# sshaoshuai/PointRCNN

Measured on AMD Instinct MI355X. Metric: KITTI frames/sec, RPN inference end-to-end (16384 pts/frame, bs32 per GPU), higher is better.
Workload: dtype f32 via split-bf16x6 MFMA (every fp32 operand cut exactly into 3 bf16 pieces, 6 bf16 MFMA products per fp32 product, fp32 accumulate: fp32-grade, measured error 2.9e-7 of sum|x||w| vs 3.0e-7 for the fp32-MFMA kernel; hoisted grouped layers on the split kernel too, unhoisted grouped first layers (xyz; 1 GPU; Full RPN PointNet++ backbone (4 SA-MSG + 4 FP) + cls/reg heads, tools/cfgs/default.yaml, 16384 pts/frame, batch 32 per GPU, random-init weights, eval-mode BN; frames_per_gpu=32, npoints=16384, parallelism=frames sharded, dp1, launch=hipGraph replay, streams=20, hw_queues=4, proposal_layer=normal, clouds=uniform, group_dedup=True, roi_dedup=True

## Files before the change

pointrcnn_amd/csrc/grid.hip:

```cpp
#include "grid_layout.h"

#define GRID_BUILD_THREADS 1024

__device__ __forceinline__ const int32_t* grid_cells(const void* g, size_t fb, int b) { return (const int32_t*)((const char*)g + fb * b + sizeof(GridHeader)); }
__device__ __forceinline__ const float4* grid_points(const void* g, size_t fb, int b) {
    size_t off = (sizeof(GridHeader) + (size_t)(GRID_CELLS_MAX + 1) * 4 + 15) & ~(size_t)15;
    return (const float4*)((const char*)g + fb * b + off);
}

__device__ __forceinline__ int cell_coord(float v, float o, float inv, int dim) {
    float t = (v - o) * inv;
    t = fminf(fmaxf(t, 0.0f), (float)(dim - 1));
    return (int)t;
}

__device__ __forceinline__ float block_reduce(float v, bool is_min, float* scratch) {
    const int lane = threadIdx.x & 63, wave = threadIdx.x >> 6, nw = blockDim.x >> 6;
#pragma unroll
    for (int d = 32; d >= 1; d >>= 1) {
        float o = __shfl_xor(v, d, 64);
        v = is_min ? fminf(v, o) : fmaxf(v, o);
    }
    __syncthreads();
    if (lane == 0) scratch[wave] = v;
    __syncthreads();
    float r = scratch[0];
    for (int w = 1; w < nw; w++) r = is_min ? fminf(r, scratch[w]) : fmaxf(r, scratch[w]);
    return r;
}

__device__ __forceinline__ float block_reduce_sum(float v, float* scratch) {
    const int lane = threadIdx.x & 63, wave = threadIdx.x >> 6, nw = blockDim.x >> 6;
#pragma unroll
    for (int d = 32; d >= 1; d >>= 1) v += __shfl_xor(v, d, 64);
    __syncthreads();
    if (lane == 0) scratch[wave] = v;
    __syncthreads();
    float r = 0.f;
    for (int w = 0; w < nw; w++) r += scratch[w];
    __syncthreads();
    return r;
}

__global__ __launch_bounds__(GRID_BUILD_THREADS) void grid_build_kernel(const float* __restrict__ xyz, int N, float min_cell, int dim,
                                                                        void* grid, size_t fb) {
    extern __shared__ int cnt[];
    const int ncell = dim * dim, per_thread = ncell / GRID_BUILD_THREADS;
    __shared__ float red[16];
    __shared__ int wsum[16];
    const int b = blockIdx.x, tid = threadIdx.x;
    const float* __restrict__ p = xyz + (size_t)b * N * 3;
    GridHeader* H = (GridHeader*)grid_header(grid, fb, b);
    int32_t* cstart = (int32_t*)grid_cells(grid, fb, b);
    float4* sorted = (float4*)grid_points(grid, fb, b);
    float mnx = INFINITY, mxx = -INFINITY, mnz = INFINITY, mxz = -INFINITY;
    for (int i = tid; i < N; i += GRID_BUILD_THREADS) {
        float x = p[i * 3], z = p[i * 3 + 2];
        if (fabsf(x) < INFINITY && fabsf(z) < INFINITY) {
            mnx = fminf(mnx, x); mxx = fmaxf(mxx, x); mnz = fminf(mnz, z); mxz = fmaxf(mxz, z);
        }
    }
    mnx = block_reduce(mnx, true, red); mxx = block_reduce(mxx, false, red);
    mnz = block_reduce(mnz, true, red); mxz = block_reduce(mxz, false, red);
    if (!(mnx <= mxx)) { mnx = mxx = 0.f; mnz = mxz = 0.f; }
    float cs = fmaxf(fmaxf(mxx - mnx, mxz - mnz) / (float)dim * 1.0001f, fmaxf(min_cell, 1e-3f));
    const float inv = 1.0f / cs;
    for (int c = tid; c < ncell; c += GRID_BUILD_THREADS) cnt[c] = 0;
    __syncthreads();
    for (int i = tid; i < N; i += GRID_BUILD_THREADS) {
        int c = cell_coord(p[i * 3 + 2], mnz, inv, dim) * dim + cell_coord(p[i * 3], mnx, inv, dim);
        atomicAdd(&cnt[c], 1);
    }
    __syncthreads();
    int ssum = 0, occ = 0;
    for (int u = 0; u < per_thread; u++) {
        const int c = cnt[tid * per_thread + u];
        ssum += c;
        occ += c > 0;
    }
    const float occupied = block_reduce_sum((float)occ, red);
    int inc = ssum;
    const int lane = tid & 63, wave = tid >> 6;
#pragma unroll
    for (int d = 1; d < 64; d <<= 1) {
        int o = __shfl_up(inc, d, 64);
        if (lane >= d) inc += o;
    }
    if (lane == 63) wsum[wave] = inc;
    __syncthreads();
    int woff = 0;
    for (int w = 0; w < wave; w++) woff += wsum[w];
    int run = woff + inc - ssum;
    for (int u = 0; u < per_thread; u++) {
        const int c = cnt[tid * per_thread + u];
        cstart[tid * per_thread + u] = run;
        cnt[tid * per_thread + u] = run;
        run += c;
    }
    if (tid == GRID_BUILD_THREADS - 1) cstart[ncell] = run;
    if (tid == 0) {
        H->x0 = mnx; H->z0 = mnz; H->inv_cs = inv; H->cs = cs; H->dim = dim;
        const float side = 2.0f * min_cell * inv + 1.0f;
        H->cand = (float)N / fmaxf(occupied, 1.0f) * side * side;
        H->pad1 = H->pad2 = 0;
    }
    __syncthreads();
    for (int i = tid; i < N; i += GRID_BUILD_THREADS) {
        float x = p[i * 3], y = p[i * 3 + 1], z = p[i * 3 + 2];
        int c = cell_coord(z, mnz, inv, dim) * dim + cell_coord(x, mnx, inv, dim);
        int pos = atomicAdd(&cnt[c], 1);
        sorted[pos] = make_float4(x, y, z, __int_as_float(i));
    }
}

#define GBQ_THREADS 64

__device__ __forceinline__ int insert_sorted(int* list, int stride, int cnt, int cap, int k) {
    if (cnt == cap) {
        if (k >= list[(cap - 1) * stride]) return cnt;
        cnt = cap - 1;
    }
    int pos = cnt;
    while (pos > 0 && list[(pos - 1) * stride] > k) { list[pos * stride] = list[(pos - 1) * stride]; pos--; }
    list[pos * stride] = k;
    return cnt + 1;
}

template <bool DUAL>
__global__ __launch_bounds__(GBQ_THREADS) void grid_ball_query_kernel(const void* __restrict__ grid, size_t fb,
                                                                     const float* __restrict__ new_xyz, int M, float ra,
                                                                     float r2a, int nsa, int32_t* __restrict__ idxa, float rb,
                                                                     float r2b, int nsb, int32_t* __restrict__ idxb, int N,
                                                                     int skip_dense) {
    extern __shared__ int lists[];
    const int b = blockIdx.y, tid = threadIdx.x;
    const int m = blockIdx.x * GBQ_THREADS + tid;
    if (m >= M) return;
    const GridHeader H = *grid_header(grid, fb, b);
    if (skip_dense && grid_frame_dense(H, N)) return;
    const int32_t* __restrict__ cstart = grid_cells(grid, fb, b);
    const float4* __restrict__ pts = grid_points(grid, fb, b);
    const float* q = new_xyz + ((size_t)b * M + m) * 3;
    const float qx = q[0], qy = q[1], qz = q[2];
    int* la = lists + tid;
    int* lb = lists + nsa * GBQ_THREADS + tid;
    int cnta = 0, cntb = 0;
    const float rmax = DUAL ? fmaxf(ra, rb) : ra;
    const float r2max = DUAL ? fmaxf(r2a, r2b) : r2a;
    const float rs = rmax * 1.001f + 1e-6f;
    if (qx == qx && qz == qz && r2max > 0.0f) {
        const int dim = H.dim;
        const int cx0 = cell_coord(qx - rs, H.x0, H.inv_cs, dim), cx1 = cell_coord(qx + rs, H.x0, H.inv_cs, dim);
        const int cz0 = cell_coord(qz - rs, H.z0, H.inv_cs, dim), cz1 = cell_coord(qz + rs, H.z0, H.inv_cs, dim);
        for (int cz = cz0; cz <= cz1; cz++) {
            const int beg = cstart[cz * dim + cx0], end = cstart[cz * dim + cx1 + 1];
            for (int t = beg; t < end; t++) {
                const float4 c = pts[t];
                const float d = sqdist3(qx, qy, qz, c.x, c.y, c.z);
                if (d < r2max) {
                    const int k = __float_as_int(c.w);
                    if (d < r2a) cnta = insert_sorted(la, GBQ_THREADS, cnta, nsa, k);
                    if (DUAL && d < r2b) cntb = insert_sorted(lb, GBQ_THREADS, cntb, nsb, k);
                }
            }
        }
    }
    int32_t* oa = idxa + ((size_t)b * M + m) * nsa;
    const int fa = cnta ? la[0] : 0;
    for (int s = 0; s < nsa; s++) oa[s] = s < cnta ? la[s * GBQ_THREADS] : fa;
    if (DUAL) {
        int32_t* ob = idxb + ((size_t)b * M + m) * nsb;
        const int fbk = cntb ? lb[0] : 0;
        for (int s = 0; s < nsb; s++) ob[s] = s < cntb ? lb[s * GBQ_THREADS] : fbk;
    }
}

template <typename T> struct __attribute__((packed, aligned(4))) Trip { T a, b, c; };

#define GNN_THREADS 256
__global__ __launch_bounds__(GNN_THREADS) void grid_three_nn_kernel(const void* __restrict__ grid, size_t fb,
                                                                    const float* __restrict__ unknown, int n,
                                                                    float* __restrict__ dist2, int32_t* __restrict__ idx,
                                                                    float* __restrict__ weight) {
    const int b = blockIdx.y;
    const int i = blockIdx.x * GNN_THREADS + threadIdx.x;
    if (i >= n) return;
    const GridHeader H = *grid_header(grid, fb, b);
    const int32_t* __restrict__ cstart = grid_cells(grid, fb, b);
    const float4* __restrict__ pts = grid_points(grid, fb, b);
    const float* u = unknown + ((size_t)b * n + i) * 3;
    const float ux = u[0], uy = u[1], uz = u[2];
    float b1 = INFINITY, b2 = INFINITY, b3 = INFINITY;
    int i1 = 0, i2 = 0, i3 = 0;
    const int GD = H.dim;
    auto visit = [&](int cz, int cxa, int cxb) __attribute__((always_inline)) {
        const int beg = cstart[cz * GD + cxa], end = cstart[cz * GD + cxb + 1];
        for (int t = beg; t < end; t++) {
            const float4 c = pts[t];
            const float dd = sqdist3(ux, uy, uz, c.x, c.y, c.z);
            const int k = __float_as_int(c.w);
            if (dd < b3 || (dd == b3 && k < i3 && dd < INFINITY)) {
                const bool lt1 = dd < b1 || (dd == b1 && k < i1);
                const bool lt2 = lt1 || dd < b2 || (dd == b2 && k < i2);
                b3 = lt2 ? b2 : dd; i3 = lt2 ? i2 : k;
                b2 = lt1 ? b1 : (lt2 ? dd : b2); i2 = lt1 ? i1 : (lt2 ? k : i2);
                b1 = lt1 ? dd : b1; i1 = lt1 ? k : i1;
            }
        }
    };
    const bool finite_q = fabsf(ux) < INFINITY && fabsf(uz) < INFINITY;
    if (finite_q) {
        const float fx = (ux - H.x0) * H.inv_cs, fz = (uz - H.z0) * H.inv_cs;
        const int qcx = (int)floorf(fminf(fmaxf(fx, -1.0f), (float)GD)), qcz = (int)floorf(fminf(fmaxf(fz, -1.0f), (float)GD));
        for (int R = 0;; R++) {
            const int x0 = qcx - R, x1 = qcx + R, z0 = qcz - R, z1 = qcz + R;
            const int cxa = max(x0, 0), cxb = min(x1, GD - 1);
            if (cxa <= cxb) {
                if (z0 >= 0 && z0 < GD) visit(z0, cxa, cxb);
                if (R > 0 && z1 >= 0 && z1 < GD) visit(z1, cxa, cxb);
            }
            if (R > 0) {
                const int za = max(z0 + 1, 0), zb = min(z1 - 1, GD - 1);
                for (int cz = za; cz <= zb; cz++) {
                    if (x0 >= 0 && x0 < GD) visit(cz, x0, x0);
                    if (x1 >= 0 && x1 < GD) visit(cz, x1, x1);
                }
            }
            if (x0 <= 0 && z0 <= 0 && x1 >= GD - 1 && z1 >= GD - 1) break;
            float lb = INFINITY;
            if (x0 > 0) lb = fminf(lb, ux - (H.x0 + (float)x0 * H.cs));
            if (x1 < GD - 1) lb = fminf(lb, (H.x0 + (float)(x1 + 1) * H.cs) - ux);
            if (z0 > 0) lb = fminf(lb, uz - (H.z0 + (float)z0 * H.cs));
            if (z1 < GD - 1) lb = fminf(lb, (H.z0 + (float)(z1 + 1) * H.cs) - uz);
            lb = lb * 0.999f - 1e-4f * H.cs;
            if (lb > 0.0f && b3 < lb * lb) break;
        }
    }
    const size_t o = ((size_t)b * n + i) * 3;
    *reinterpret_cast<Trip<float>*>(dist2 + o) = Trip<float>{b1, b2, b3};
    *reinterpret_cast<Trip<int32_t>*>(idx + o) = Trip<int32_t>{i1, i2, i3};
    if (weight) {
        float r0 = 1.0f / (sqrtf(b1) + 1e-8f);
        float r1 = 1.0f / (sqrtf(b2) + 1e-8f);
        float r2 = 1.0f / (sqrtf(b3) + 1e-8f);
        float s = (r0 + r1) + r2;
        *reinterpret_cast<Trip<float>*>(weight + o) = Trip<float>{r0 / s, r1 / s, r2 / s};
    }
}

PRCNN_API size_t prcnn_grid_bytes(int B, int N) {
    if (B <= 0 || N <= 0) return 0;
    return grid_frame_bytes(N) * (size_t)B;
}

PRCNN_API int prcnn_grid_build(const float* xyz, int B, int N, float min_cell, int cells_per_axis, void* grid, size_t grid_bytes,
                               prcnn_stream_t stream) {
    PRCNN_REQUIRE(B >= 0 && N > 0 && min_cell >= 0.0f, "prcnn_grid_build: bad shape B=%d N=%d min_cell=%g", B, N, (double)min_cell);
    PRCNN_REQUIRE(cells_per_axis == 64 || cells_per_axis == 128, "prcnn_grid_build: cells_per_axis must be 64 or 128, got %d", cells_per_axis);
    if (B == 0) return PRCNN_OK;
    PRCNN_REQUIRE(xyz && grid, "prcnn_grid_build: null pointer");
    PRCNN_REQUIRE(((uintptr_t)grid & 15) == 0, "prcnn_grid_build: grid buffer must be 16-byte aligned");
    PRCNN_REQUIRE(grid_bytes >= prcnn_grid_bytes(B, N), "prcnn_grid_build: buffer %zu < %zu bytes", grid_bytes, prcnn_grid_bytes(B, N));
    static PrcnnLdsLimit attr;
    if (!attr.raise((const void*)grid_build_kernel, GRID_CELLS_MAX * 4))
        return prcnn_fail(PRCNN_EHIP, "prcnn_grid_build: cannot raise the dynamic LDS limit");
    hipLaunchKernelGGL(grid_build_kernel, dim3(B), dim3(GRID_BUILD_THREADS), (size_t)cells_per_axis * cells_per_axis * 4, (hipStream_t)stream,
                       xyz, N, min_cell, cells_per_axis, grid, grid_frame_bytes(N));
    PRCNN_LAUNCH_CHECK("prcnn_grid_build");
    return PRCNN_OK;
}

PRCNN_API int prcnn_ball_query2_grid(const void* grid, const float* xyz, const float* new_xyz, int B, int N, int M, float radius_a,
                                     int nsample_a, int32_t* idx_a, float radius_b, int nsample_b, int32_t* idx_b, prcnn_stream_t stream) {
    const bool dual = nsample_b > 0;
    PRCNN_REQUIRE(B >= 0 && N > 0 && M >= 0 && nsample_a > 0 && nsample_b >= 0, "prcnn_ball_query2_grid: bad shape");
    if (B == 0 || M == 0) return PRCNN_OK;
    PRCNN_REQUIRE(grid && new_xyz && idx_a && (!dual || idx_b), "prcnn_ball_query2_grid: null pointer");
    const size_t lds = (size_t)(nsample_a + nsample_b) * GBQ_THREADS * sizeof(int);
    PRCNN_REQUIRE(lds <= 64 * 1024, "prcnn_ball_query2_grid: nsample %d+%d too large for the LDS hit lists", nsample_a, nsample_b);
    dim3 g(prcnn_divup(M, GBQ_THREADS), B);
    const float r2a = radius_a * radius_a, r2b = radius_b * radius_b;
    if (dual)
        hipLaunchKernelGGL(grid_ball_query_kernel<true>, g, dim3(GBQ_THREADS), lds, (hipStream_t)stream, grid, grid_frame_bytes(N),
                           new_xyz, M, radius_a, r2a, nsample_a, idx_a, radius_b, r2b, nsample_b, idx_b, N, xyz ? 1 : 0);
    else
        hipLaunchKernelGGL(grid_ball_query_kernel<false>, g, dim3(GBQ_THREADS), lds, (hipStream_t)stream, grid, grid_frame_bytes(N),
                           new_xyz, M, radius_a, r2a, nsample_a, idx_a, 0.f, 0.f, 0, (int32_t*)nullptr, N, xyz ? 1 : 0);
    PRCNN_LAUNCH_CHECK("prcnn_ball_query2_grid");
    if (xyz) return prcnn_launch_ball_query_scan(xyz, new_xyz, B, N, M, radius_a, nsample_a, idx_a, radius_b, nsample_b, idx_b, grid,
                                                 (hipStream_t)stream);
    return PRCNN_OK;
}

PRCNN_API int prcnn_three_nn_grid(const void* grid, const float* unknown, int B, int n, int m, float* dist2, int32_t* idx,
                                  float* weight, prcnn_stream_t stream) {
    PRCNN_REQUIRE(B >= 0 && n >= 0 && m > 0, "prcnn_three_nn_grid: bad shape B=%d n=%d m=%d", B, n, m);
    if (B == 0 || n == 0) return PRCNN_OK;
    PRCNN_REQUIRE(grid && unknown && dist2 && idx, "prcnn_three_nn_grid: null pointer");
    hipLaunchKernelGGL(grid_three_nn_kernel, dim3(prcnn_divup(n, GNN_THREADS), B), dim3(GNN_THREADS), 0, (hipStream_t)stream, grid,
                       grid_frame_bytes(m), unknown, n, dist2, idx, weight);
    PRCNN_LAUNCH_CHECK("prcnn_three_nn_grid");
    return PRCNN_OK;
}
```

pointrcnn_amd/csrc/grid_layout.h:

```cpp
#pragma once
#include "common.h"

#define GRID_DIM_MAX 128
#define GRID_CELLS_MAX (GRID_DIM_MAX * GRID_DIM_MAX)

struct GridHeader {
    float x0, z0, inv_cs, cs;
    int dim;
    float cand;
    int pad1, pad2;
};
static inline size_t grid_frame_bytes(int N) {
    size_t b = sizeof(GridHeader) + (size_t)(GRID_CELLS_MAX + 1) * 4;
    b = (b + 15) & ~(size_t)15;
    return b + (size_t)N * 16;
}
__device__ __forceinline__ const GridHeader* grid_header(const void* g, size_t fb, int b) { return (const GridHeader*)((const char*)g + fb * b); }
__device__ __forceinline__ bool grid_frame_dense(const GridHeader& H, int N) { return H.cand > (float)N * (1.0f / 32.0f); }

int prcnn_launch_ball_query_scan(const float* xyz, const float* new_xyz, int B, int N, int M, float radius_a, int nsample_a,
                                 int32_t* idx_a, float radius_b, int nsample_b, int32_t* idx_b, const void* grid, hipStream_t s);
```

pointrcnn_amd/csrc/neighbor.hip:

```cpp
#include "grid_layout.h"

#define BQ_THREADS 64
#define NN_THREADS 256
#define NB_CHUNK 1024

typedef float f32x2 __attribute__((ext_vector_type(2)));

__device__ __forceinline__ f32x2 pair_sqdist(const float* rec, f32x2 qx, f32x2 qy, f32x2 qz) {
    float4 a = *reinterpret_cast<const float4*>(rec);
    f32x2 z = *reinterpret_cast<const f32x2*>(rec + 4);
    f32x2 dx = qx - (f32x2){a.x, a.y}, dy = qy - (f32x2){a.z, a.w}, dz = qz - z;
    return (dx * dx + dy * dy) + dz * dz;
}

template <bool DUAL>
__global__ __launch_bounds__(BQ_THREADS) void ball_query_kernel(const float* __restrict__ xyz,
                                                                const float* __restrict__ new_xyz, int N, int M,
                                                                float r2a, int nsa, int32_t* __restrict__ idxa,
                                                                float r2b, int nsb, int32_t* __restrict__ idxb,
                                                                const void* __restrict__ grid, size_t grid_fb) {
    __shared__ __attribute__((aligned(16))) float spts[NB_CHUNK * 4];
    const int b = blockIdx.y, tid = threadIdx.x;
    if (grid && !grid_frame_dense(*grid_header(grid, grid_fb, b), N)) return;
    const int m = blockIdx.x * BQ_THREADS + tid;
    const bool valid = m < M;
    const float* __restrict__ p = xyz + (size_t)b * N * 3;
    float qx = 0.f, qy = 0.f, qz = 0.f;
    if (valid) {
        const float* q = new_xyz + ((size_t)b * M + m) * 3;
        qx = q[0]; qy = q[1]; qz = q[2];
    }
    const f32x2 qx2 = {qx, qx}, qy2 = {qy, qy}, qz2 = {qz, qz};
    int32_t* oa = idxa + ((size_t)b * M + (valid ? m : 0)) * nsa;
    int32_t* ob = DUAL ? idxb + ((size_t)b * M + (valid ? m : 0)) * nsb : nullptr;
    int cnta = 0, cntb = 0, firsta = 0, firstb = 0;
    const float r2max = DUAL ? fmaxf(r2a, r2b) : r2a;
    bool done = !valid;

    constexpr int PER_LANE = NB_CHUNK * 3 / BQ_THREADS;
    float pre[PER_LANE];
    auto fetch_chunk = [&](int c0) {
        const int cnt3 = min(NB_CHUNK, N - c0) * 3;
        const float* src = p + (size_t)c0 * 3;
#pragma unroll
        for (int u = 0; u < PER_LANE; u++) {
            int i = tid + u * BQ_THREADS;
            pre[u] = i < cnt3 ? src[i] : INFINITY;
        }
    };
    auto store_chunk = [&]() {
#pragma unroll
        for (int u = 0; u < PER_LANE; u++) {
            int i = tid + u * BQ_THREADS;
            int pt = i / 3, c = i - pt * 3;
            spts[(pt >> 1) * 8 + c * 2 + (pt & 1)] = pre[u];
        }
    };
    fetch_chunk(0);
    for (int c0 = 0; c0 < N; c0 += NB_CHUNK) {
        if (__all(done)) break;
        __syncthreads();
        store_chunk();
        __syncthreads();
        if (c0 + NB_CHUNK < N) fetch_chunk(c0 + NB_CHUNK);
        if (!done) {
            for (int i0 = 0; i0 < NB_CHUNK; i0 += 8) {
                f32x2 d2[4];
                bool any = false;
#pragma unroll
                for (int u = 0; u < 4; u++) {
                    d2[u] = pair_sqdist(spts + (i0 / 2 + u) * 8, qx2, qy2, qz2);
                    any |= (d2[u].x < r2max) | (d2[u].y < r2max);
                }
                if (any) {
#pragma unroll
                    for (int u = 0; u < 8; u++) {
                        float d = (u & 1) ? d2[u >> 1].y : d2[u >> 1].x;
                        if (d < r2max) {
                            int k = c0 + i0 + u;
                            if (d < r2a && cnta < nsa) {
                                if (cnta == 0) firsta = k;
                                oa[cnta++] = k;
                            }
                            if (DUAL && d < r2b && cntb < nsb) {
                                if (cntb == 0) firstb = k;
                                ob[cntb++] = k;
                            }
                        }
                    }
                    if (cnta >= nsa && (!DUAL || cntb >= nsb)) { done = true; break; }
                }
            }
        }
    }
    if (valid) {
        for (int s = cnta; s < nsa; s++) oa[s] = firsta;
        if (DUAL)
            for (int s = cntb; s < nsb; s++) ob[s] = firstb;
    }
}

__global__ __launch_bounds__(NN_THREADS) void three_nn_kernel(const float* __restrict__ unknown,
                                                              const float* __restrict__ known, int n, int m,
                                                              float* __restrict__ dist2, int32_t* __restrict__ idx,
                                                              float* __restrict__ weight) {
    __shared__ __attribute__((aligned(16))) float spts[NB_CHUNK * 4];
    const int b = blockIdx.y, tid = threadIdx.x;
    const int i = blockIdx.x * NN_THREADS + tid;
    const bool valid = i < n;
    const float* __restrict__ p = known + (size_t)b * m * 3;
    float ux = 0.f, uy = 0.f, uz = 0.f;
    if (valid) {
        const float* u = unknown + ((size_t)b * n + i) * 3;
        ux = u[0]; uy = u[1]; uz = u[2];
    }
    const f32x2 ux2 = {ux, ux}, uy2 = {uy, uy}, uz2 = {uz, uz};
    float b1 = INFINITY, b2 = INFINITY, b3 = INFINITY;
    int i1 = 0, i2 = 0, i3 = 0;
    constexpr int PER_LANE = NB_CHUNK * 3 / NN_THREADS;
    float pre[PER_LANE];
    auto fetch_chunk = [&](int c0) {
        const int cnt3 = min(NB_CHUNK, m - c0) * 3;
        const float* src = p + (size_t)c0 * 3;
#pragma unroll
        for (int u = 0; u < PER_LANE; u++) {
            int e = tid + u * NN_THREADS;
            pre[u] = e < cnt3 ? src[e] : INFINITY;
        }
    };
    fetch_chunk(0);
    for (int c0 = 0; c0 < m; c0 += NB_CHUNK) {
        __syncthreads();
#pragma unroll
        for (int u = 0; u < PER_LANE; u++) {
            int e = tid + u * NN_THREADS;
            int pt = e / 3, c = e - pt * 3;
            spts[(pt >> 1) * 8 + c * 2 + (pt & 1)] = pre[u];
        }
        __syncthreads();
        if (c0 + NB_CHUNK < m) fetch_chunk(c0 + NB_CHUNK);
        for (int j0 = 0; j0 < NB_CHUNK; j0 += 8) {
            f32x2 d[4];
            bool any = false;
#pragma unroll
            for (int u = 0; u < 4; u++) {
                d[u] = pair_sqdist(spts + (j0 / 2 + u) * 8, ux2, uy2, uz2);
                any |= (d[u].x < b3) | (d[u].y < b3);
            }
            if (any) {
#pragma unroll
                for (int u = 0; u < 8; u++) {
                    float dd = (u & 1) ? d[u >> 1].y : d[u >> 1].x;
                    if (dd < b3) {
                        int k = c0 + j0 + u;
                        if (dd < b1) { b3 = b2; i3 = i2; b2 = b1; i2 = i1; b1 = dd; i1 = k; }
                        else if (dd < b2) { b3 = b2; i3 = i2; b2 = dd; i2 = k; }
                        else { b3 = dd; i3 = k; }
                    }
                }
            }
        }
    }
    if (valid) {
        size_t o = ((size_t)b * n + i) * 3;
        dist2[o] = b1; dist2[o + 1] = b2; dist2[o + 2] = b3;
        idx[o] = i1; idx[o + 1] = i2; idx[o + 2] = i3;
        if (weight) {
            float r0 = 1.0f / (sqrtf(b1) + 1e-8f);
            float r1 = 1.0f / (sqrtf(b2) + 1e-8f);
            float r2 = 1.0f / (sqrtf(b3) + 1e-8f);
            float s = (r0 + r1) + r2;
            weight[o] = r0 / s; weight[o + 1] = r1 / s; weight[o + 2] = r2 / s;
        }
    }
}

static int ball_query_impl(const float* xyz, const float* new_xyz, int B, int N, int M, float ra, int nsa, int32_t* ia,
                           float rb, int nsb, int32_t* ib, bool dual, hipStream_t s, const void* dense_grid = nullptr) {
    PRCNN_REQUIRE(B >= 0 && N > 0 && M >= 0 && nsa > 0 && (!dual || nsb > 0),
                  "prcnn_ball_query: bad shape B=%d N=%d M=%d nsample=%d/%d", B, N, M, nsa, nsb);
    if (B == 0 || M == 0) return PRCNN_OK;
    PRCNN_REQUIRE(xyz && new_xyz && ia && (!dual || ib), "prcnn_ball_query: null pointer");
    dim3 grid(prcnn_divup(M, BQ_THREADS), B);
    float r2a = ra * ra, r2b = rb * rb;
    const size_t gfb = grid_frame_bytes(N);
    if (dual)
        hipLaunchKernelGGL(ball_query_kernel<true>, grid, dim3(BQ_THREADS), 0, s, xyz, new_xyz, N, M, r2a, nsa, ia, r2b,
                           nsb, ib, dense_grid, gfb);
    else
        hipLaunchKernelGGL(ball_query_kernel<false>, grid, dim3(BQ_THREADS), 0, s, xyz, new_xyz, N, M, r2a, nsa, ia,
                           0.f, 0, (int32_t*)nullptr, dense_grid, gfb);
    PRCNN_LAUNCH_CHECK("prcnn_ball_query");
    return PRCNN_OK;
}

int prcnn_launch_ball_query_scan(const float* xyz, const float* new_xyz, int B, int N, int M, float radius_a, int nsample_a,
                                 int32_t* idx_a, float radius_b, int nsample_b, int32_t* idx_b, const void* grid, hipStream_t s) {
    return ball_query_impl(xyz, new_xyz, B, N, M, radius_a, nsample_a, idx_a, radius_b, nsample_b, idx_b, nsample_b > 0, s, grid);
}

PRCNN_API int prcnn_ball_query(const float* xyz, const float* new_xyz, int B, int N, int M, float radius, int nsample,
                               int32_t* idx, prcnn_stream_t stream) {
    return ball_query_impl(xyz, new_xyz, B, N, M, radius, nsample, idx, 0.f, 0, nullptr, false, (hipStream_t)stream);
}

PRCNN_API int prcnn_ball_query2(const float* xyz, const float* new_xyz, int B, int N, int M, float radius_a,
                                int nsample_a, int32_t* idx_a, float radius_b, int nsample_b, int32_t* idx_b,
                                prcnn_stream_t stream) {
    return ball_query_impl(xyz, new_xyz, B, N, M, radius_a, nsample_a, idx_a, radius_b, nsample_b, idx_b, true,
                           (hipStream_t)stream);
}

PRCNN_API int prcnn_three_nn(const float* unknown, const float* known, int B, int n, int m, float* dist2, int32_t* idx,
                             float* weight, prcnn_stream_t stream) {
    PRCNN_REQUIRE(B >= 0 && n >= 0 && m > 0, "prcnn_three_nn: bad shape B=%d n=%d m=%d", B, n, m);
    if (B == 0 || n == 0) return PRCNN_OK;
    PRCNN_REQUIRE(unknown && known && dist2 && idx, "prcnn_three_nn: null pointer");
    hipLaunchKernelGGL(three_nn_kernel, dim3(prcnn_divup(n, NN_THREADS), B), dim3(NN_THREADS), 0, (hipStream_t)stream,
                       unknown, known, n, m, dist2, idx, weight);
    PRCNN_LAUNCH_CHECK("prcnn_three_nn");
    return PRCNN_OK;
}
```

pointrcnn_amd/opbench.py:

```python
import argparse
import json
import os

import numpy as np
import torch

from . import ops, rpn

HBM_PEAK_GBS = 8000.0
HBM_COPY_GBS = 6300.0
MFMA_F32_PEAK_TF = 157.3


def timeit(fn, iters=20, warm=3):
    for _ in range(warm):
        fn()
    s, e = torch.cuda.Event(enable_timing=True), torch.cuda.Event(enable_timing=True)
    torch.cuda.synchronize()
    s.record()
    for _ in range(iters):
        fn()
    e.record()
    torch.cuda.synchronize()
    return s.elapsed_time(e) / iters * 1e-3


def emit(name, shape, sec, **kw):
    d = {"op": name, "shape": shape, "avg_launch_us": round(sec * 1e6, 1)}
    if "bytes" in kw:
        comp = kw.get("compulsory", kw["bytes"])
        gbs, agbs = comp / sec / 1e9, kw["bytes"] / sec / 1e9
        d.update(bound="hbm", compulsory_MB=round(comp / 1e6, 1), achieved_GBps=round(gbs, 1),
                 frac_of_8TBps=round(gbs / HBM_PEAK_GBS, 3), frac_of_6p3TBps_copy_ceiling=round(gbs / HBM_COPY_GBS, 3),
                 algorithmic_MB=round(kw["bytes"] / 1e6, 1), algorithmic_GBps=round(agbs, 1),
                 served_from_cache=bool(agbs > HBM_COPY_GBS))
    if "kernels" in kw:
        d["kernels"] = [[k, int(g)] for k, g in kw["kernels"]]
    if "pairs" in kw:
        d.update(bound="valu", pair_evals=kw["pairs"], achieved_Gpairs_per_s=round(kw["pairs"] / sec / 1e9, 1))
    if "flops" in kw:
        tf = kw["flops"] / sec / 1e12
        d.update(bound="mfma", achieved_TFLOPs=round(tf, 2), frac_of_peak=round(tf / MFMA_F32_PEAK_TF, 3))
    d.update(kw.get("parts", {}))
    print(json.dumps(d), flush=True)


def train_scene_rows(dev, B=16, n_raw=115000, npoints=16384, D=2000):
    import numpy as np
    from . import kitti_input
    r = np.random.default_rng(7)
    dbb = (r.random((D, 7)) * [60., .8, 60., .3, .3, 1., 6.28] + [-30., 1.2, 5., 1.4, 1.5, 3.4, -3.14]).astype(np.float32)
    npd = r.integers(5, 400, D)
    gdb = kitti_input.GTDatabase.from_arrays(dbb, np.zeros(D, np.float32), [r.random((int(n), 3)).astype(np.float32) + dbb[i, :3] for i, n in enumerate(npd)],
                                             [r.random(int(n)).astype(np.float32) for n in npd], device=dev)
    calib = kitti_input.Calibration.from_text(kitti_input.KITTI_CALIB_TXT)
    scans = [kitti_input.synthetic_scan(n_raw + 97 * b, seed=900 + b) for b in range(B)]
    labels = [(r.random((12, 7)) * [60., .8, 60., .3, .3, 1., 6.28] + [-30., 1.2, 5., 1.4, 1.5, 3.4, -3.14]).astype(np.float32) for _ in range(B)]
    planes = [[0.0, -1.0, 0.0, 1.65]] * B
    prep = kitti_input.TrainScenePreparer(npoints=npoints, gt_database=gdb, device=dev)
    packed = prep.pack(scans, [calib] * B, [(375, 1242)] * B, labels, [np.zeros(12, np.float32)] * B, labels, planes)
    t = {k: (v.to(dev) if isinstance(v, torch.Tensor) else v) for k, v in packed.items()}
    inf = kitti_input.ScenePreparer(npoints=npoints, device=dev)

    def row(name, shape, fn):
        ts = [timeit(fn) for _ in range(5)]
        d = {"op": name, "shape": shape, "avg_launch_us": round(sum(ts) / 5 * 1e6, 1), "min_us": round(min(ts) * 1e6, 1),
             "max_us": round(max(ts) * 1e6, 1)}
        print(json.dumps(d), flush=True)
        return sum(ts) / 5
    shape = "B%d ~%dk raw npoints %d D%d" % (B, n_raw // 1000, npoints, D)
    out = prep(packed, 5)
    total = row("train_scene_prepare", shape + " (H2D excluded: sampler + train scene + labels)", lambda: _train_scene_device(prep, t, packed["max_points"], 5))
    parts = row("scene_prepare", shape, lambda: ops.scene_prepare(t["raw"], t["offsets"], packed["max_points"], t["calib"], t["img_hw"], inf.scope, npoints, 5))
    parts += row("gt_aug_sample", "B%d G12 D%d" % (B, D), lambda: gdb.sample(t["all_gt_boxes3d"], t["num_all_gt"], t["planes"], seed=5))
    nv = int(out["nvalid"].max())
    xyz, inten = torch.randn(B, nv, 3, device=dev) * 20.0, torch.rand(B, nv, device=dev)
    npts, nint = torch.randn(B, 4000, 3, device=dev), torch.rand(B, 4000, device=dev)
    acc = gdb.sample(t["all_gt_boxes3d"], t["num_all_gt"], t["planes"], seed=5)["boxes3d"]
    parts += row("gt_aug_edit", "B%d N%d K%d P4000 (random cloud)" % (B, nv, acc.shape[1]), lambda: ops.gt_aug_edit(xyz, inten, acc, npts, nint))
    parts += row("rpn_labels", "B%d N%d G%d" % (B, npoints, out["gt_boxes3d"].shape[1]), lambda: ops.rpn_labels(out["pts_rect"], out["gt_boxes3d"], out["num_gt"]))
    print(json.dumps({"op": "train_scene_prepare vs separate passes", "train_scene_prepare_us": round(total * 1e6, 1),
                      "sum_of_separate_passes_us": round(parts * 1e6, 1)}), flush=True)


def _train_scene_device(prep, t, max_points, seed):
    acc = prep.db.sample(t["all_gt_boxes3d"], t["num_all_gt"], t["planes"], prep.extra_num, prep.rand_num, prep.apply_prob,
                         [prep.scope[0:2], prep.scope[2:4], prep.scope[4:6]], prep.try_times, prep.max_accept, seed)
    out = ops.train_scene_prepare(t["raw"], t["offsets"], max_points, t["calib"], t["img_hw"], prep.scope, prep.npoints, seed,
                                  t["gt_boxes3d"], t["gt_alpha"], t["num_gt"], acc, prep.db, prep.methods, prep.prob, prep.rot_range)
    return ops.rpn_labels(out["pts_rect"], out["gt_boxes3d"], out["num_gt"])


def gt_database_row(dev, B=8, n_raw=120000, nbox=8):
    import numpy as np
    from . import kitti_input
    r = np.random.default_rng(17)
    calib = kitti_input.Calibration.from_text(kitti_input.KITTI_CALIB_TXT)
    scans = [kitti_input.synthetic_scan(n_raw, seed=300 + b) for b in range(B)]
    boxes = np.zeros((B, nbox, 7), np.float32)
    for b, sc in enumerate(scans):
        rect = kitti_input.lidar_to_rect_host(sc, calib.lidar_to_rect_matrix())
        c = rect[r.choice(np.nonzero((rect[:, 2] > 5) & (rect[:, 2] < 40) & (np.abs(rect[:, 0]) < 20))[0], nbox)]
        boxes[b] = np.concatenate([c[:, :1], c[:, 1:2] + 0.8, c[:, 2:3], np.tile([[1.6, 1.7, 4.0]], (nbox, 1)), r.uniform(-3.14, 3.14, (nbox, 1))], 1)
    pk = kitti_input.pack_scans(scans, [calib] * B, [(375, 1242)] * B, pin=False)
    raw, off, cal = pk["raw"].to(dev), pk["offsets"].to(dev), pk["calib"].to(dev)
    bx, nb = torch.from_numpy(boxes).to(dev), torch.full((B,), nbox, dtype=torch.int32, device=dev)
    P = ops.gt_database_build(raw, off, pk["max_points"], cal, bx, nb)[2].shape[0]
    emit("gt_database_build", "B%d x %d raw points x %d boxes (%d points kept; includes the host read of the total)" % (B, n_raw, nbox, P),
         timeit(lambda: ops.gt_database_build(raw, off, pk["max_points"], cal, bx, nb)),
         bytes=2 * raw.numel() * 4 + P * 20 + B * nbox * 4, kernels=[("gtdb_kernel", 0), ("gtdb_scan_kernel", 0)])


def aug_scene_row(dev, B=8, n_raw=120000, G=12, D=2000):
    import numpy as np
    from . import kitti_input
    r = np.random.default_rng(27)
    calib = kitti_input.Calibration.from_text(kitti_input.KITTI_CALIB_TXT)
    box = lambda n: (r.random((n, 7)) * [60., .8, 60., .3, .3, 1., 6.28] + [-30., 1.2, 5., 1.4, 1.5, 3.4, -3.14]).astype(np.float32)
    dbb, npd = box(D), r.integers(5, 400, D)
    gdb = kitti_input.GTDatabase.from_arrays(dbb, np.zeros(D, np.float32), [r.random((int(n), 3)).astype(np.float32) + dbb[i, :3] for i, n in enumerate(npd)],
                                             [r.random(int(n)).astype(np.float32) for n in npd], hard_ratio=0.0, device=dev)
    pk = kitti_input.pack_scans([kitti_input.synthetic_scan(n_raw, seed=400 + b) for b in range(B)], [calib] * B, [(375, 1242)] * B, pin=False)
    raw, off, cal, hw = (pk[k].to(dev) for k in ("raw", "offsets", "calib", "img_hw"))
    gt = torch.from_numpy(np.stack([box(G) for _ in range(B)])).to(dev)
    planes = torch.tensor([[0.0, -1.0, 0.0, 1.65]] * B, dtype=torch.float64, device=dev)
    ids = torch.arange(10000, 10000 + B, dtype=torch.int32, device=dev)
    scope = kitti_input.aug_scene_scope("Car")
    sample = lambda: ops.aug_scene_sample(gt, None, planes, ids, gdb.boxes, gdb.npts, scope, 5)
    acc = sample()
    emit("aug_scene_sample", "B%d G%d D%d (%d objects accepted)" % (B, G, D, int(acc["count"].sum())), timeit(sample), kernels=[("augs_sample_kernel", 0)])
    build = lambda: ops.aug_scene_build(raw, off, pk["max_points"], cal, hw, scope, acc, gdb.points, gdb.intensity, gdb.offsets)
    rows = build()[2].shape[0]
    emit("aug_scene_build", "B%d x %d raw points (%d rows out; includes the host read of the total)" % (B, n_raw, rows), timeit(build),
         bytes=2 * raw.numel() * 4 + rows * 20, kernels=[("augs_tile_kernel", 0), ("augs_scan_kernel", 0), ("augs_paste_kernel", 0)])


def rpn_loss_rows(dev, B=16, N=16384, rounds=5):
    from . import train_functions as tf
    g = torch.Generator().manual_seed(7)
    u = torch.rand(B, N, generator=g)
    lab = torch.where(u < 0.03, 1, torch.where(u < 0.13, -1, 0)).to(dev)
    reg_lab = (torch.rand(B, N, 7, generator=g) * torch.tensor([6., 2., 6., 1., 1., 2., 6.28]) + torch.tensor([-3., -1., -3., 1., 1., 3., -3.14])).to(dev)
    cls = torch.randn(B, N, 1, generator=g).to(dev).requires_grad_(True)
    reg = torch.randn(B, N, 76, generator=g).to(dev).requires_grad_(True)

    def step(fused):
        cls.grad = reg.grad = None
        tf.get_rpn_loss(cls, reg, lab, reg_lab, fused=fused).backward()
    times = {False: [], True: []}
    for _ in range(rounds):
        for fused in (False, True):
            times[fused].append(timeit(lambda: step(fused)))
    n_fg, npts = int((lab > 0).sum()), B * N
    floor = 2 * (npts * (8 + 28 + 4) + n_fg * 76 * 4) + npts * 77 * 4
    for fused in (False, True):
        t = sorted(times[fused])
        d = {"op": "rpn_loss fwd+bwd (%s)" % ("fused" if fused else "composed"), "shape": "B%d N%d C76, %d foreground rows" % (B, N, n_fg),
             "median_us": round(t[len(t) // 2] * 1e6, 1), "min_us": round(t[0] * 1e6, 1), "max_us": round(t[-1] * 1e6, 1)}
        if fused:
            d.update(traffic_floor_MB=round(floor / 1e6, 1), floor_GBps_at_median=round(floor / t[len(t) // 2] / 1e9, 1))
        print(json.dumps(d), flush=True)


def optimizer_rows(dev, rounds=5):
    from . import point_rcnn
    from .optim import OneCycleAdam
    g = torch.Generator().manual_seed(3)
    for name, net in (("rpn.RPN()", rpn.RPN()), ("rcnn_net", point_rcnn.PointRCNN(mode="TRAIN").rcnn_net)):
        shapes = [p.shape for p in net.parameters() if p.requires_grad]
        opts = {}
        for fused in (False, True):
            ps = [torch.nn.Parameter((torch.randn(s, generator=g) * 0.1).to(dev)) for s in shapes]
            for p in ps:
                p.grad = (torch.randn(p.shape, generator=g) * 0.01).to(dev)
            opts[fused] = OneCycleAdam(ps, 10000, fused=fused)
        times = {False: [], True: []}
        for _ in range(rounds):
            for fused in (False, True):
                times[fused].append(timeit(opts[fused].step))
        n = sum(int(torch.Size(s).numel()) for s in shapes)
        for fused in (False, True):
            t = sorted(times[fused])
            d = {"op": "optimizer step (%s)" % ("fused" if fused else "composed"), "shape": "%s: %d tensors, %d elements" % (name, len(shapes), n),
                 "median_us": round(t[len(t) // 2] * 1e6, 1), "min_us": round(t[0] * 1e6, 1), "max_us": round(t[-1] * 1e6, 1)}
            if fused:
                d.update(traffic_floor_MB=round(32 * n / 1e6, 2), floor_GBps_at_median=round(32 * n / t[len(t) // 2] / 1e9, 1),
                         table_uploads=opts[True].table_uploads)
            print(json.dumps(d), flush=True)


def rcnn_offline_rows(dev, B=4, M=300, G=12, R=64, N=16384, C=128, S=512):
    import numpy as np
    from . import kitti_input, rcnn
    rng = np.random.default_rng(12)

    def scene(M):
        gt = (rng.random((B, G, 7)) * [60., .3, 50., .3, .3, .8, 6.28] + [-30., 1.4, 8., 1.4, 1.5, 3.5, -3.14]).astype(np.float32)
        roi = (rng.random((B, M, 7)) * [70., .4, 60., .3, .3, 1., 6.28] + [-35., 1.3, 4., 1.4, 1.5, 3.4, -3.14]).astype(np.float32)
        for j in range(G):
            near = gt[:, j:j + 1] + rng.normal(0, 1, (B, 8, 7)) * [.1, .03, .1, .03, .03, .06, .03]
            hard = gt[:, j:j + 1] + rng.normal(0, 1, (B, 8, 7)) * [.1, .03, .1, .03, .03, .06, .03]
            hard[..., 0] += np.cos(gt[:, j:j + 1, 6]) * 0.5 * gt[:, j:j + 1, 5]
            hard[..., 2] -= np.sin(gt[:, j:j + 1, 6]) * 0.5 * gt[:, j:j + 1, 5]
            roi[:, 16 * j:16 * j + 8], roi[:, 16 * j + 8:16 * j + 16] = near, hard
        return roi, gt
    roi, gt = scene(M)
    ctr = gt[np.arange(B)[:, None], rng.integers(0, G, (B, N))][..., :3]
    xyz = (ctr + rng.normal(0, 1, (B, N, 3)) * [1.8, .6, 1.8] - [0, .8, 0]).astype(np.float32)
    frames = [{"sample_id": b, "rpn_xyz": xyz[b], "rpn_features": rng.normal(0, 1, (N, C)).astype(np.float32),
               "rpn_intensity": rng.random(N).astype(np.float32), "seg_mask": (rng.random(N) > 0.5).astype(np.float32),
               "roi_boxes3d": roi[b], "roi_scores": np.zeros(M, np.float32), "gt_boxes3d": gt[b]} for b in range(B)]
    cfg = type("Cfg", (rcnn.RCNNConfig,), dict(ROI_SAMPLE_JIT=False, ROI_PER_IMAGE=R, NUM_POINTS=S))
    prep = kitti_input.RCNNOfflinePreparer(cfg, dev)
    d = prep._upload(prep.pack(frames, pin=False))
    out = prep(d, seed=3)
    assert not out["status"].any() and (out["cls_label"] == 1).any() and (out["cls_label"] == 0).any()
    thr = (cfg.REG_FG_THRESH, cfg.CLS_FG_THRESH, cfg.CLS_BG_THRESH)
    sample = lambda: ops.rcnn_offline_sample(d["roi_boxes3d"], d["num_roi"], d["gt_boxes3d"], d["num_gt"], R, seed=3, frame_ids=d["frame_ids"])
    s = sample()
    _, feat = prep._point_features(d)
    pooled, empty = rcnn.roipool3d_gpu(d["rpn_xyz"], feat, s["rois"], cfg.POOL_EXTRA_WIDTH, S)
    t_all = timeit(lambda: prep(d, seed=3))
    t_s = timeit(sample)
    t_p = timeit(lambda: rcnn.roipool3d_gpu(d["rpn_xyz"], feat, s["rois"], cfg.POOL_EXTRA_WIDTH, S))
    t_f = timeit(lambda: ops.rcnn_offline_finish(pooled, s, empty, thr, prep.aug_methods, prep.flip_prob, cfg.AUG_ROT_RANGE, 3, d["frame_ids"]))
    emit("rcnn_offline_batch", "bs%d M%d G%d R%d N%d S%d C%d (upload excluded; includes the (B,N,%d) feature concat)" % (B, M, G, R, N, S, C, 2 + C),
         t_all, bytes=B * R * S * (5 + C) * 4, parts={"sample_us": round(t_s * 1e6, 1), "pool_us": round(t_p * 1e6, 1), "finish_us": round(t_f * 1e6, 1)})
    big, bgt = scene(4096)
    T = lambda a, dt=None: torch.from_numpy(np.ascontiguousarray(a, dt)).to(dev)
    br, bg, bn, bm = T(big), T(bgt), T(np.full(B, 4096), np.int32), T(np.full(B, G), np.int32)
    emit("rcnn_offline_sample", "bs%d M4096 G%d R%d (the RoI cap)" % (B, G, R), timeit(lambda: ops.rcnn_offline_sample(br, bn, bg, bm, R, seed=3)),
         pairs=B * 4096 * G)


def rcnn_loss_rows(dev, R=256, rounds=5):
    from . import train_functions as tf
    from .rcnn import RCNNConfig
    g = torch.Generator().manual_seed(9)
    u = torch.rand(R, generator=g)
    mean = torch.tensor(tf.RPNLossConfig.MEAN_SIZE)
    roi, gt = torch.zeros(R, 7), torch.zeros(R, 7)
    roi[:, 3:6] = (torch.rand(R, 3, generator=g) * 0.4 + 0.8) * mean
    gt[:, 0:3] = (torch.rand(R, 3, generator=g) * 2.8 - 1.4) * torch.tensor([1.0, 0.3, 1.0])
    gt[:, 3:6] = (torch.rand(R, 3, generator=g) * 0.4 + 0.8) * mean
    gt[:, 6] = torch.rand(R, generator=g) * 2.0 - 1.0
    ret = {"rcnn_cls": (torch.randn(R, 1, generator=g) * 2).to(dev).requires_grad_(True),
           "rcnn_reg": torch.randn(R, 46, generator=g).to(dev).requires_grad_(True),
           "cls_label": torch.where(u < 0.3, 1, torch.where(u < 0.45, -1, 0)).to(dev),
           "reg_valid_mask": (torch.rand(R, generator=g) < 0.35).long().to(dev), "roi_boxes3d": roi.to(dev), "gt_of_rois": gt.to(dev)}

    def step(fused):
        ret["rcnn_cls"].grad = ret["rcnn_reg"].grad = None
        tf.get_rcnn_loss(ret, RCNNConfig, fused=fused).backward()
    times = {False: [], True: []}
    for _ in range(rounds):
        for fused in (False, True):
            times[fused].append(timeit(lambda: step(fused)))
    for fused in (False, True):
        t = sorted(times[fused])
        print(json.dumps({"op": "rcnn_loss fwd+bwd (%s)" % ("fused" if fused else "composed"),
                          "shape": "R%d C46, %d regressed rows" % (R, int(ret["reg_valid_mask"].sum())),
                          "median_us": round(t[len(t) // 2] * 1e6, 1), "min_us": round(t[0] * 1e6, 1), "max_us": round(t[-1] * 1e6, 1)}), flush=True)


def eval_stats_rows(dev, B=32, shapes=((100, 12), (512, 24)), N=16384, rounds=5):
    from .eval_stats import THRESH_LIST, EvalStats
    gq = torch.Generator().manual_seed(21)
    span, base = torch.tensor([60., .8, 60., .3, .3, 1., 6.28]), torch.tensor([-30., 1.2, 5., 1.4, 1.5, 3.4, -3.14])
    seg = (torch.rand(B, N, generator=gq) < 0.2).float().to(dev)
    label = (torch.rand(B, N, generator=gq) < 0.2).long().to(dev)
    for M, G in shapes:
        gt = torch.rand(B, G, 7, generator=gq) * span + base
        gt[:, G - G // 4:] = 0
        near = gt[:, torch.randint(0, G - G // 4, (M,), generator=gq)] + torch.randn(B, M, 7, generator=gq) * 0.2
        far = torch.rand(B, M, 7, generator=gq) * span + base
        rois = torch.where(torch.rand(B, M, 1, generator=gq) < 0.5, near, far).to(dev).contiguous()
        pred = (rois + torch.randn(B, M, 7, generator=gq).to(dev) * 0.05).contiguous()
        gt = gt.to(dev)
        num = torch.randint(0, 20, (B,), generator=gq, dtype=torch.int32).to(dev)
        stats = EvalStats("joint", dev)

        def composed():
            total = [0] * 5, [0] * 5
            total_gt = final_total = 0
            total_rpn_iou = 0.0
            for k in range(B):
                cur = gt[k]
                n = cur.shape[0] - 1
                while n >= 0 and cur[n].sum().item() == 0:
                    n -= 1
                if n >= 0:
                    cur = cur[:n + 1].contiguous()
                    for which, boxes in enumerate((pred[k], rois[k])):
                        gt_max_iou, _ = ops.boxes_iou3d(boxes, cur).max(dim=0)
                        for idx, thresh in enumerate(THRESH_LIST):
                            total[which][idx] += (gt_max_iou > thresh).sum().item()
                    total_gt += cur.shape[0]
                fg_mask = label > 0
                correct = ((seg == label) & fg_mask).sum().float()
                union = fg_mask.sum().float() + (seg > 0).sum().float() - correct
                total_rpn_iou += (correct / torch.clamp(union, min=1.0)).item()
                final_total += int(num[k].item())
            return total, total_gt, total_rpn_iou, final_total

        def device():
            stats.update(rois, gt, pred_boxes3d=pred, det_num=num, seg_result=seg, rpn_cls_label=label)
        times = {"composed": [], "device": []}
        for _ in range(rounds):
            times["composed"].append(timeit(composed))
            times["device"].append(timeit(device))
        for route in ("composed", "device"):
            t = sorted(times[route])
            print(json.dumps({"op": "eval_stats (%s)" % route, "shape": "B%d M%d G%d N%d joint" % (B, M, G, N),
                              "median_us": round(t[len(t) // 2] * 1e6, 1), "min_us": round(t[0] * 1e6, 1), "max_us": round(t[-1] * 1e6, 1),
                              "launches_per_update": 2 if route == "device" else None}), flush=True)


class _P2:
    P2 = np.array([[721.5377, 0, 609.5593, 44.85728], [0, 721.5377, 172.854, 0.2163791], [0, 0, 1, 0.002745884]], np.float32)


def _kitti_like_detections(B, M, g):
    span = torch.tensor([50., 1.4, 68., .76, .81, 1.94, 6.28])
    base = torch.tensor([-25., .8, 2., 1.22, 1.30, 3.11, -3.14])
    boxes = torch.rand(B, M, 7, generator=g) * span + base
    boxes[:, :4, 2] = torch.rand(B, 4, generator=g) * 1.8 + 1.2
    scores = torch.randn(B, M, generator=g) * 3
    keep = torch.stack([torch.randperm(M, generator=g) for _ in range(B)]).to(torch.int32)
    num = torch.randint(M // 2, M + 1, (B,), generator=g, dtype=torch.int32)
    return boxes, scores, keep, num


def _tmpfs_dir():
    import tempfile
    return tempfile.mkdtemp(prefix="prcnn_opbench_", dir="/dev/shm" if os.path.isdir("/dev/shm") else None)


def result_writer_rows(dev, B=32, Ms=(100, 512), rounds=5, iters=5):
    import shutil
    import time
    from . import kitti_output
    g = torch.Generator().manual_seed(33)
    for M in Ms:
        boxes, scores, keep, num = (t.to(dev).contiguous() for t in _kitti_like_detections(B, M, g))
        calibs, shapes, ids = [_P2] * B, [(375, 1242, 3)] * B, list(range(B))
        writer = kitti_output.DeviceResultWriter(dev)
        dirs = {"host": _tmpfs_dir(), "device": _tmpfs_dir()}

        def host():
            kitti_output.write_detections(boxes, scores, keep, num, ids, calibs, shapes, dirs["host"])

        def device():
            writer.write(writer.format(boxes, scores, keep, num, calibs, shapes), ids, dirs["device"])

        def window(fn):
            fn()
            torch.cuda.synchronize()
            t0 = time.perf_counter()
            for _ in range(iters):
                fn()
            return (time.perf_counter() - t0) / iters
        times = {"host": [], "device": []}
        try:
            for _ in range(rounds):
                times["host"].append(window(host))
                times["device"].append(window(device))
            lines = sum(open("%s/%06d.txt" % (dirs["device"], i)).read().count("\n") for i in ids)
        finally:
            for d in dirs.values():
                shutil.rmtree(d, ignore_errors=True)
        P2 = torch.from_numpy(_P2.P2).double().reshape(1, 12).repeat(B, 1).to(dev)
        hw = torch.tensor([[375, 1242]] * B, dtype=torch.int32, device=dev)
        out = ops.kitti_result_text(boxes, scores, P2, hw, keep=keep, num=num)
        kernel = timeit(lambda: ops.kitti_result_text(boxes, scores, P2, hw, keep=keep, num=num, out=out))
        faster = all(d < h for d, h in zip(times["device"], times["host"]))
        for route in ("host", "device"):
            t = sorted(times[route])
            print(json.dumps({"op": "result_writer (%s)" % route, "shape": "B%d M%d, %d lines" % (B, M, lines),
                              "median_ms_per_batch": round(t[len(t) // 2] * 1e3, 3), "min_ms": round(t[0] * 1e3, 3), "max_ms": round(t[-1] * 1e3, 3),
                              "rounds_ms": [round(x * 1e3, 3) for x in times[route]],
                              "kernel_us": round(kernel * 1e6, 1) if route == "device" else None,
                              "device_faster_in_every_round": faster}), flush=True)
        if not faster:
            raise AssertionError("result_writer: the device route was not faster than the host route in every round at M=%d: %s" % (M, times))


def eval_loop_rows(dev, B=16, nbatches=3, rounds=5):
    import shutil
    import time
    from . import eval_stats, kitti_output
    from .point_rcnn import PointRCNN
    torch.manual_seed(0)
    model = rpn.randomize_bn_stats(PointRCNN(mode="TEST")).to(dev).eval()
    pts = rpn.synthetic_clouds(B * nbatches, 16384, device=dev)
    batches = [{"sample_id": list(range(k * B, (k + 1) * B)), "pts_input": pts[k * B:(k + 1) * B]} for k in range(nbatches)]
    writer = kitti_output.DeviceResultWriter(dev)
    times = {"host": [], "device": []}
    out = _tmpfs_dir()
    try:
        for r in range(rounds + 1):
            for route, w in (("host", None), ("device", writer)):
                torch.cuda.synchronize()
                t0 = time.perf_counter()
                eval_stats.eval_one_epoch_joint(model, batches, "%s/%s" % (out, route), lambda i: _P2, lambda i: (375, 1242, 3), writer=w)
                torch.cuda.synchronize()
                if r:
                    times[route].append(time.perf_counter() - t0)
        files = ["%s/device/final_result/data/%06d.txt" % (out, i) for i in range(B * nbatches)]
        lines = sum(open(f).read().count("\n") for f in files if os.path.exists(f))
    finally:
        shutil.rmtree(out, ignore_errors=True)
    for route in ("host", "device"):
        fps = sorted(B * nbatches / t for t in times[route])
        print(json.dumps({"op": "eval_loop joint (%s writer)" % route, "shape": "%d batches of %d frames, 16384 points, %d detections" % (nbatches, B, lines),
                          "median_frames_per_s": round(fps[len(fps) // 2], 1), "min": round(fps[0], 1), "max": round(fps[-1], 1)}), flush=True)


def main():
    ap = argparse.ArgumentParser()
    ap.add_argument("--quick", action="store_true")
    ap.add_argument("--only", default=None, help="run one row family only: eval_stats | optimizer | result_writer | eval_loop")
    args = ap.parse_args()
    dev = torch.device("cuda:0")
    if args.only == "result_writer":
        result_writer_rows(dev)
        return
    if args.only == "eval_loop":
        eval_loop_rows(dev)
        return
    if args.only == "eval_stats":
        eval_stats_rows(dev)
        return
    if args.only == "optimizer":
        optimizer_rows(dev)
        return
    B = 8 if args.quick else 32
    N = 16384
    xyz = rpn.synthetic_clouds(B, N, device=dev)
    g = torch.Generator(device="cpu").manual_seed(0)

    buf_a = torch.empty(1 << 28, dtype=torch.float32, device=dev)
    buf_b = torch.empty(1 << 28, dtype=torch.float32, device=dev)
    t_fill = timeit(lambda: buf_a.fill_(1.0), 10, 2)
    t_copy = timeit(lambda: buf_b.copy_(buf_a), 10, 2)
    print(json.dumps({"op": "stream ceilings", "shape": "1 GiB fp32", "write_only_GBps": round(buf_a.numel() * 4 / t_fill / 1e9, 1),
                      "copy_read_plus_write_GBps": round(2 * buf_a.numel() * 4 / t_copy / 1e9, 1),
                      "note": "torch fill_ / copy_ on this box; an op that writes W bytes and reads R cannot finish before W / write_only (R << W) or "
                              "(R + W) / copy (R ~ W)"}), flush=True)
    del buf_a, buf_b
    torch.cuda.empty_cache()

    emit("fps", "B%d %d->4096" % (B, N), timeit(lambda: ops.furthest_point_sample(xyz, 4096), 5, 1), pairs=B * N * 4096)
    new_xyz = ops.gather_rows(xyz, ops.furthest_point_sample(xyz, 4096))
    emit("ball_query2", "B%d N%d M4096 r(.1,.5) ns(16,32)" % (B, N),
         timeit(lambda: ops.ball_query2(0.1, 16, 0.5, 32, xyz, new_xyz)), pairs=B * N * 4096)
    emit("three_nn", "B%d n%d m4096" % (B, N), timeit(lambda: ops.three_nn(xyz, new_xyz)), pairs=B * N * 4096)

    feat = torch.randn(B, 96, 4096, device=dev)
    xyz1 = new_xyz
    nx2 = ops.gather_rows(xyz1, ops.furthest_point_sample(xyz1, 1024))
    idx = ops.ball_query(1.0, 32, xyz1, nx2)
    emit("grouping_operation", "B%d C96 N4096 M1024 ns32" % B, timeit(lambda: ops.group(feat, idx)),
         bytes=B * (1024 * 32 * 4 + 2 * 96 * 1024 * 32 * 4), compulsory=B * (1024 * 32 * 4 + 96 * 4096 * 4 + 96 * 1024 * 32 * 4),
         kernels=[("gather_pm_kernel", 0)])
    fidx = ops.furthest_point_sample(xyz1, 1024)
    emit("gather_operation", "B%d C96 N4096 M1024" % B, timeit(lambda: ops.gather(feat, fidx)),
         bytes=B * (1024 * 4 + 2 * 96 * 1024 * 4), compulsory=B * (1024 * 4 + 2 * 96 * 1024 * 4), kernels=[("gather_kernel", B * 1024)])
    d2, i3, w3 = ops.three_nn(xyz, xyz1, want_weight=True)
    kf = torch.randn(B, 256, 4096, device=dev)
    emit("three_interpolate", "B%d C256 m4096 n%d" % (B, N), timeit(lambda: ops.three_interpolate(kf, i3, w3)),
         bytes=B * (N * 24 + 3 * 256 * N * 4 + 256 * N * 4), compulsory=B * (N * 24 + 256 * 4096 * 4 + 256 * N * 4),
         kernels=[("three_interp", 0)])

    def rois_for(x, M, seed):
        gg = torch.Generator().manual_seed(seed)
        pick = torch.randint(0, x.shape[1], (x.shape[0], M), generator=gg).to(dev)
        ctr = torch.gather(x, 1, pick.unsqueeze(-1).expand(-1, -1, 3))
        sz = torch.tensor([1.6 + 2, 1.7 + 2, 4.0 + 2], device=dev).expand(x.shape[0], M, 3)
        ry = (torch.rand(x.shape[0], M, 1, generator=gg).to(dev) - 0.5) * 6.28
        return torch.cat([ctr[..., 0:1], ctr[..., 1:2] + 1.8, ctr[..., 2:3], sz, ry], 2).contiguous()

    pf = torch.randn(B, N, 130, device=dev)
    rois = rois_for(xyz, 100, 1)
    emit("roipool3d", "B%d N%d M100 C130 S512 (config 3)" % (B, N), timeit(lambda: ops.roipool3d(xyz, rois, pf, 512)),
         bytes=B * 2 * 100 * 512 * 133 * 4, compulsory=B * (100 * 512 * 133 * 4 + N * 133 * 4),
         kernels=[("roipool3d_kernel", B * 100 * 256)] + [("rp_bins_%s_kernel" % k, 0) for k in ("extent", "count", "scan", "fill")])
    if not args.quick:
        Bd, Nd, Md = 8, 65536, 512
        xd = rpn.synthetic_clouds(Bd, Nd, seed0=500, device=dev)
        pfd = torch.randn(Bd, Nd, 130, device=dev)
        rd = rois_for(xd, Md, 2)
        emit("roipool3d", "B%d N%d M%d C130 S512 (config 5 dense)" % (Bd, Nd, Md),
             timeit(lambda: ops.roipool3d(xd, rd, pfd, 512), 5, 1), bytes=Bd * 2 * Md * 512 * 133 * 4,
             compulsory=Bd * (Md * 512 * 133 * 4 + Nd * 133 * 4),
             kernels=[("roipool3d_kernel", Bd * Md * 256)] + [("rp_bins_%s_kernel" % k, 0) for k in ("extent", "count", "scan", "fill")])
        del xd, pfd, rd

    ab = rois_for(xyz, 15, 3)
    npts, nint = torch.randn(B, 4000, 3, device=dev), torch.rand(B, 4000, device=dev)
    inten = torch.rand(B, N, device=dev)
    emit("gt_aug_edit", "B%d N%d K15 P4000" % (B, N), timeit(lambda: ops.gt_aug_edit(xyz, inten, ab, npts, nint)),
         bytes=B * (2 * N * 16 + 2 * 4000 * 16))

    from . import kitti_input
    gq = torch.Generator().manual_seed(11)
    cb = torch.rand(256, 7, generator=gq) * torch.tensor([60., 1., 60., 1., 1., 3., 6.28]) + torch.tensor([-30., 1., 5., 1., 1., 2., -3.14])
    hw, hl, c, s_ = cb[:, 4:5] / 2, cb[:, 5:6] / 2, torch.cos(cb[:, 6:7]), torch.sin(cb[:, 6:7])
    lx = torch.cat([hl, hl, -hl, -hl] * 2, 1); lz = torch.cat([hw, -hw, -hw, hw] * 2, 1)
    ly = torch.cat([torch.zeros(256, 4), -cb[:, 3:4].expand(-1, 4)], 1)
    corners = torch.stack([cb[:, 0:1] + lx * c + lz * s_, cb[:, 1:2] + ly, cb[:, 2:3] - lx * s_ + lz * c], 2).to(dev).contiguous()
    emit("corner_iou3d", "256 x 256 pairs", timeit(lambda: ops.corner_iou3d(corners, corners)), pairs=256 * 256)
    Bs, D = 16, 2000
    dbb = (torch.rand(D, 7, generator=gq) * torch.tensor([60., .8, 60., .3, .3, 1., 6.28]) + torch.tensor([-30., 1.2, 5., 1.4, 1.5, 3.4, -3.14]))
    npd = torch.randint(5, 400, (D,), generator=gq)
    gdb = kitti_input.GTDatabase.from_arrays(dbb.numpy(), torch.zeros(D).numpy(), [torch.zeros(int(n), 3).numpy() for n in npd],
                                             [torch.zeros(int(n)).numpy() for n in npd], device=dev)
    sg = (torch.rand(Bs, 12, 7, generator=gq) * torch.tensor([60., .8, 60., .3, .3, 1., 6.28]) + torch.tensor([-30., 1.2, 5., 1.4, 1.5, 3.4, -3.14])).to(dev)
    ngt = torch.full((Bs,), 12, dtype=torch.int32, device=dev)
    planes = torch.tensor([[0.0, -1.0, 0.0, 1.65]] * Bs, dtype=torch.float64, device=dev)
    emit("gt_aug_sample", "B%d G12 D%d (default.yaml: 10-14 extra, 100 tries)" % (Bs, D),
         timeit(lambda: gdb.sample(sg, ngt, planes, seed=5)))

    rcnn_offline_rows(dev)

    train_scene_rows(dev, B=4 if args.quick else 16)

    gt_database_row(dev)

    aug_scene_row(dev)

    rpn_loss_rows(dev)
    rcnn_loss_rows(dev)
    optimizer_rows(dev)
    eval_stats_rows(dev)
    result_writer_rows(dev)
    eval_loop_rows(dev)

    c = torch.rand(6300, 2, generator=g) * torch.tensor([80.0, 70.0])
    s = torch.rand(6300, 2, generator=g) * torch.tensor([0.5, 1.5]) + torch.tensor([0.8, 1.7])
    bev = torch.cat([c - s, c + s, (torch.rand(6300, 1, generator=g) - 0.5) * 6.28], 1).to(dev)
    emit("nms_normal", "N6300 thr0.8", timeit(lambda: ops.nms_sorted(bev, 0.8, rotated=False)), pairs=6300 * 6299 // 2)
    emit("nms_rotated", "N6300 thr0.8", timeit(lambda: ops.nms_sorted(bev, 0.8, rotated=True), 5, 1), pairs=6300 * 6299 // 2)

    reg = torch.randn(B * N, 76, device=dev)
    anchor = (1.52563191462, 1.62856739989, 3.88311640418)
    emit("decode_bbox_target", "B%d N%d C76" % (B, N),
         timeit(lambda: ops.decode_bbox_target(xyz.view(-1, 3), reg, 3.0, 0.5, 12, anchor, y_to_bottom=True)),
         bytes=B * N * (76 + 3 + 7) * 4, kernels=[("decode_kernel", 0)])
    gg = torch.Generator().manual_seed(3)
    nfg = int(N * 0.4)
    obj = torch.rand(B, 24, 7, generator=gg) * torch.tensor([70., .4, 62., .3, .3, 1., 6.28]) + torch.tensor([-35., .8, 4., 1.4, 1.5, 3.4, -3.14])
    own = torch.randint(0, 24, (B, nfg), generator=gg)
    fgb = torch.gather(obj, 1, own.unsqueeze(-1).expand(-1, -1, 7)) + torch.randn(B, nfg, 7, generator=gg) * torch.tensor([.08, .03, .12, .03, .03, .06, .03])
    bgb = torch.rand(B, N - nfg, 7, generator=gg) * torch.tensor([80., 4., 70., 1., .8, 2., 6.28]) + torch.tensor([-40., -1., .2, 1., 1.2, 3., -3.14])
    boxes3d = torch.cat([fgb, bgb], 1).to(dev).contiguous()
    scores = torch.cat([torch.randn(B, nfg, generator=gg) + 2.5, torch.randn(B, N - nfg, generator=gg) - 3.0], 1).to(dev)
    for rot in (False, True):
        emit("proposal_layer(%s nms 0.8, 6300/2700 -> 70/30)" % ("rotated" if rot else "normal"), "B%d N%d" % (B, N),
             timeit(lambda: ops.proposal_layer(scores, boxes3d, (6300, 2700), (70, 30), 0.8, rotated=rot)), pairs=B * N)
    rb = boxes3d[:, :100].contiguous()
    rs = scores[:, :100].contiguous()
    emit("nms_batched(rotated 0.1)", "B%d M100" % B, timeit(lambda: ops.nms_batched(rb, rs, None, 0.1, True)), pairs=B * 100)

    model = rpn.randomize_bn_stats(rpn.RPN()).to(dev).eval()
    sa2 = model.backbone_net.SA_modules[1]
    f1 = torch.randn(B, 96, 4096, device=dev)
    with torch.no_grad():
        sec = timeit(lambda: sa2(xyz1, f1))
    macs = 1024 * (16 * (99 * 64 + 64 * 64 + 64 * 128) + 32 * (99 * 64 + 64 * 96 + 96 * 128))
    emit("SA2 module (fps+ball_query+fused MLP chains)", "B%d 4096->1024" % B, sec, flops=2.0 * B * macs)


if __name__ == "__main__":
    main()
```

Baseline: 14180 frames/s.

## Rework grid build, dense-frame ball query, LDS-staged three_nn and multi-lane queries

The grid build now caches each thread's points in registers, reduces the four bounds in a single block reduction, and uses int4 vectorised prefix scans. Dense frames no longer take a separate scan pass: the grid ball query runs the brute-force scan block inline. Grid three_nn stages points and cell offsets in LDS with larger blocks, and each ring step visits two cell ranges together. Brute-force ball query and three_nn split one query across several lanes when there are few queries, merging results with shuffles. This adds code paths and register/LDS pressure.

```diff
diff --git a/pointrcnn_amd/csrc/grid.hip b/pointrcnn_amd/csrc/grid.hip
--- a/pointrcnn_amd/csrc/grid.hip
+++ b/pointrcnn_amd/csrc/grid.hip
@@ -1,6 +1,7 @@
 #include "grid_layout.h"
 
 #define GRID_BUILD_THREADS 1024
+#define GRID_BUILD_REG_PTS 16
 
 __device__ __forceinline__ const int32_t* grid_cells(const void* g, size_t fb, int b) { return (const int32_t*)((const char*)g + fb * b + sizeof(GridHeader)); }
 __device__ __forceinline__ const float4* grid_points(const void* g, size_t fb, int b) {
@@ -14,19 +15,21 @@
     return (int)t;
 }
 
-__device__ __forceinline__ float block_reduce(float v, bool is_min, float* scratch) {
+__device__ __forceinline__ void block_reduce_bounds(float& mnx, float& mxx, float& mnz, float& mxz, float* scratch) {
     const int lane = threadIdx.x & 63, wave = threadIdx.x >> 6, nw = blockDim.x >> 6;
 #pragma unroll
     for (int d = 32; d >= 1; d >>= 1) {
-        float o = __shfl_xor(v, d, 64);
-        v = is_min ? fminf(v, o) : fmaxf(v, o);
-    }
-    __syncthreads();
-    if (lane == 0) scratch[wave] = v;
-    __syncthreads();
-    float r = scratch[0];
-    for (int w = 1; w < nw; w++) r = is_min ? fminf(r, scratch[w]) : fmaxf(r, scratch[w]);
-    return r;
+        mnx = fminf(mnx, __shfl_xor(mnx, d, 64)); mxx = fmaxf(mxx, __shfl_xor(mxx, d, 64));
+        mnz = fminf(mnz, __shfl_xor(mnz, d, 64)); mxz = fmaxf(mxz, __shfl_xor(mxz, d, 64));
+    }
+    __syncthreads();
+    if (lane == 0) { scratch[wave * 4] = mnx; scratch[wave * 4 + 1] = mxx; scratch[wave * 4 + 2] = mnz; scratch[wave * 4 + 3] = mxz; }
+    __syncthreads();
+    mnx = scratch[0]; mxx = scratch[1]; mnz = scratch[2]; mxz = scratch[3];
+    for (int w = 1; w < nw; w++) {
+        mnx = fminf(mnx, scratch[w * 4]); mxx = fmaxf(mxx, scratch[w * 4 + 1]);
+        mnz = fminf(mnz, scratch[w * 4 + 2]); mxz = fmaxf(mxz, scratch[w * 4 + 3]);
+    }
 }
 
 __device__ __forceinline__ float block_reduce_sum(float v, float* scratch) {
@@ -44,39 +47,62 @@
 
 __global__ __launch_bounds__(GRID_BUILD_THREADS) void grid_build_kernel(const float* __restrict__ xyz, int N, float min_cell, int dim,
                                                                         void* grid, size_t fb) {
-    extern __shared__ int cnt[];
-    const int ncell = dim * dim, per_thread = ncell / GRID_BUILD_THREADS;
-    __shared__ float red[16];
+    extern __shared__ __attribute__((aligned(16))) int cnt[];
+    const int ncell = dim * dim, per_thread4 = ncell / GRID_BUILD_THREADS / 4;
+    __shared__ float red[4 * GRID_BUILD_THREADS / 64];
     __shared__ int wsum[16];
     const int b = blockIdx.x, tid = threadIdx.x;
     const float* __restrict__ p = xyz + (size_t)b * N * 3;
     GridHeader* H = (GridHeader*)grid_header(grid, fb, b);
     int32_t* cstart = (int32_t*)grid_cells(grid, fb, b);
     float4* sorted = (float4*)grid_points(grid, fb, b);
+    const bool inreg = N <= GRID_BUILD_REG_PTS * GRID_BUILD_THREADS;
+    float px[GRID_BUILD_REG_PTS], py[GRID_BUILD_REG_PTS], pz[GRID_BUILD_REG_PTS];
+    if (inreg) {
+#pragma unroll
+        for (int u = 0; u < GRID_BUILD_REG_PTS; u++) {
+            const int i = tid + u * GRID_BUILD_THREADS;
+            if (i < N) {
+                const Trip<float> v = *reinterpret_cast<const Trip<float>*>(p + (size_t)i * 3);
+                px[u] = v.a; py[u] = v.b; pz[u] = v.c;
+            }
+        }
+    }
+    auto for_points = [&](auto&& f) __attribute__((always_inline)) {
+        if (inreg) {
+#pragma unroll
+            for (int u = 0; u < GRID_BUILD_REG_PTS; u++) {
+                const int i = tid + u * GRID_BUILD_THREADS;
+                if (i < N) f(i, px[u], py[u], pz[u]);
+            }
+        } else {
+            for (int i = tid; i < N; i += GRID_BUILD_THREADS) f(i, p[i * 3], p[i * 3 + 1], p[i * 3 + 2]);
+        }
+    };
     float mnx = INFINITY, mxx = -INFINITY, mnz = INFINITY, mxz = -INFINITY;
-    for (int i = tid; i < N; i += GRID_BUILD_THREADS) {
-        float x = p[i * 3], z = p[i * 3 + 2];
+    for_points([&](int, float x, float, float z) {
         if (fabsf(x) < INFINITY && fabsf(z) < INFINITY) {
             mnx = fminf(mnx, x); mxx = fmaxf(mxx, x); mnz = fminf(mnz, z); mxz = fmaxf(mxz, z);
         }
-    }
-    mnx = block_reduce(mnx, true, red); mxx = block_reduce(mxx, false, red);
-    mnz = block_reduce(mnz, true, red); mxz = block_reduce(mxz, false, red);
+    });
+    block_reduce_bounds(mnx, mxx, mnz, mxz, red);
     if (!(mnx <= mxx)) { mnx = mxx = 0.f; mnz = mxz = 0.f; }
     float cs = fmaxf(fmaxf(mxx - mnx, mxz - mnz) / (float)dim * 1.0001f, fmaxf(min_cell, 1e-3f));
     const float inv = 1.0f / cs;
-    for (int c = tid; c < ncell; c += GRID_BUILD_THREADS) cnt[c] = 0;
-    __syncthreads();
-    for (int i = tid; i < N; i += GRID_BUILD_THREADS) {
-        int c = cell_coord(p[i * 3 + 2], mnz, inv, dim) * dim + cell_coord(p[i * 3], mnx, inv, dim);
+    for (int c = tid; c < ncell / 4; c += GRID_BUILD_THREADS) reinterpret_cast<int4*>(cnt)[c] = make_int4(0, 0, 0, 0);
+    __syncthreads();
+    for_points([&](int, float x, float, float z) {
+        int c = cell_coord(z, mnz, inv, dim) * dim + cell_coord(x, mnx, inv, dim);
         atomicAdd(&cnt[c], 1);
-    }
-    __syncthreads();
+    });
+    __syncthreads();
+    int4* cnt4 = reinterpret_cast<int4*>(cnt) + tid * per_thread4;
+    int4* cstart4 = reinterpret_cast<int4*>(cstart) + tid * per_thread4;
     int ssum = 0, occ = 0;
-    for (int u = 0; u < per_thread; u++) {
-        const int c = cnt[tid * per_thread + u];
-        ssum += c;
-        occ += c > 0;
+    for (int u = 0; u < per_thread4; u++) {
+        const int4 c = cnt4[u];
+        ssum += (c.x + c.y) + (c.z + c.w);
+        occ += (c.x > 0) + (c.y > 0) + (c.z > 0) + (c.w > 0);
     }
     const float occupied = block_reduce_sum((float)occ, red);
     int inc = ssum;
@@ -91,11 +117,12 @@
     int woff = 0;
     for (int w = 0; w < wave; w++) woff += wsum[w];
     int run = woff + inc - ssum;
-    for (int u = 0; u < per_thread; u++) {
-        const int c = cnt[tid * per_thread + u];
-        cstart[tid * per_thread + u] = run;
-        cnt[tid * per_thread + u] = run;
-        run += c;
+    for (int u = 0; u < per_thread4; u++) {
+        const int4 c = cnt4[u];
+        const int4 st = make_int4(run, run + c.x, run + c.x + c.y, run + c.x + c.y + c.z);
+        cstart4[u] = st;
+        cnt4[u] = st;
+        run = st.w + c.w;
     }
     if (tid == GRID_BUILD_THREADS - 1) cstart[ncell] = run;
     if (tid == 0) {
@@ -105,15 +132,15 @@
         H->pad1 = H->pad2 = 0;
     }
     __syncthreads();
-    for (int i = tid; i < N; i += GRID_BUILD_THREADS) {
-        float x = p[i * 3], y = p[i * 3 + 1], z = p[i * 3 + 2];
+    for_points([&](int i, float x, float y, float z) {
         int c = cell_coord(z, mnz, inv, dim) * dim + cell_coord(x, mnx, inv, dim);
         int pos = atomicAdd(&cnt[c], 1);
         sorted[pos] = make_float4(x, y, z, __int_as_float(i));
-    }
+    });
 }
 
 #define GBQ_THREADS 64
+static_assert(GBQ_THREADS == BQ_THREADS, "a dense frame's workgroups run the scan of neighbor.hip: same block, same grid");
 
 __device__ __forceinline__ int insert_sorted(int* list, int stride, int cnt, int cap, int k) {
     if (cnt == cap) {
@@ -128,16 +155,19 @@
 
 template <bool DUAL>
 __global__ __launch_bounds__(GBQ_THREADS) void grid_ball_query_kernel(const void* __restrict__ grid, size_t fb,
+                                                                     const float* __restrict__ xyz,
                                                                      const float* __restrict__ new_xyz, int M, float ra,
                                                                      float r2a, int nsa, int32_t* __restrict__ idxa, float rb,
-                                                                     float r2b, int nsb, int32_t* __restrict__ idxb, int N,
-                                                                     int skip_dense) {
-    extern __shared__ int lists[];
+                                                                     float r2b, int nsb, int32_t* __restrict__ idxb, int N) {
+    extern __shared__ __attribute__((aligned(16))) int lists[];
     const int b = blockIdx.y, tid = threadIdx.x;
+    const GridHeader H = *grid_header(grid, fb, b);
+    if (xyz && grid_frame_dense(H, N)) {
+        ball_query_scan_block<DUAL>(reinterpret_cast<float*>(lists), xyz, new_xyz, N, M, b, blockIdx.x, r2a, nsa, idxa, r2b, nsb, idxb);
+        return;
+    }
     const int m = blockIdx.x * GBQ_THREADS + tid;
     if (m >= M) return;
-    const GridHeader H = *grid_header(grid, fb, b);
-    if (skip_dense && grid_frame_dense(H, N)) return;
     const int32_t* __restrict__ cstart = grid_cells(grid, fb, b);
     const float4* __restrict__ pts = grid_points(grid, fb, b);
     const float* q = new_xyz + ((size_t)b * M + m) * 3;
@@ -175,28 +205,22 @@
     }
 }
 
-template <typename T> struct __attribute__((packed, aligned(4))) Trip { T a, b, c; };
-
 #define GNN_THREADS 256
-__global__ __launch_bounds__(GNN_THREADS) void grid_three_nn_kernel(const void* __restrict__ grid, size_t fb,
-                                                                    const float* __restrict__ unknown, int n,
-                                                                    float* __restrict__ dist2, int32_t* __restrict__ idx,
-                                                                    float* __restrict__ weight) {
-    const int b = blockIdx.y;
-    const int i = blockIdx.x * GNN_THREADS + threadIdx.x;
-    if (i >= n) return;
-    const GridHeader H = *grid_header(grid, fb, b);
-    const int32_t* __restrict__ cstart = grid_cells(grid, fb, b);
-    const float4* __restrict__ pts = grid_points(grid, fb, b);
-    const float* u = unknown + ((size_t)b * n + i) * 3;
-    const float ux = u[0], uy = u[1], uz = u[2];
-    float b1 = INFINITY, b2 = INFINITY, b3 = INFINITY;
-    int i1 = 0, i2 = 0, i3 = 0;
+#define GNN_LDS_THREADS 1024
+#define GNN_LDS_DIM 64
+#define GNN_LDS_MAX_M 4096
+#define GNN_LDS_CELL_BYTES (((GNN_LDS_DIM * GNN_LDS_DIM + 1) * 4 + 15) & ~15)
+
+__device__ __forceinline__ void grid_three_nn_rings(const GridHeader& H, const int32_t* __restrict__ cstart, const float4* __restrict__ pts,
+                                                    float ux, float uy, float uz, float& b1, float& b2, float& b3, int& i1, int& i2,
+                                                    int& i3) {
     const int GD = H.dim;
-    auto visit = [&](int cz, int cxa, int cxb) __attribute__((always_inline)) {
-        const int beg = cstart[cz * GD + cxa], end = cstart[cz * GD + cxb + 1];
-        for (int t = beg; t < end; t++) {
-            const float4 c = pts[t];
+    auto visit2 = [&](bool oka, int cza, int cxa0, int cxa1, bool okb, int czb, int cxb0, int cxb1) __attribute__((always_inline)) {
+        const int bega = cstart[oka ? cza * GD + cxa0 : 0], enda = cstart[oka ? cza * GD + cxa1 + 1 : 0];
+        const int begb = cstart[okb ? czb * GD + cxb0 : 0], endb = cstart[okb ? czb * GD + cxb1 + 1 : 0];
+        const int na = enda - bega, nb = endb - begb;
+        for (int j = 0; j < na + nb; j++) {
+            const float4 c = pts[j < na ? bega + j : begb + (j - na)];
             const float dd = sqdist3(ux, uy, uz, c.x, c.y, c.z);
             const int k = __float_as_int(c.w);
             if (dd < b3 || (dd == b3 && k < i3 && dd < INFINITY)) {
@@ -209,42 +233,69 @@
         }
     };
     const bool finite_q = fabsf(ux) < INFINITY && fabsf(uz) < INFINITY;
-    if (finite_q) {
-        const float fx = (ux - H.x0) * H.inv_cs, fz = (uz - H.z0) * H.inv_cs;
-        const int qcx = (int)floorf(fminf(fmaxf(fx, -1.0f), (float)GD)), qcz = (int)floorf(fminf(fmaxf(fz, -1.0f), (float)GD));
-        for (int R = 0;; R++) {
-            const int x0 = qcx - R, x1 = qcx + R, z0 = qcz - R, z1 = qcz + R;
-            const int cxa = max(x0, 0), cxb = min(x1, GD - 1);
-            if (cxa <= cxb) {
-                if (z0 >= 0 && z0 < GD) visit(z0, cxa, cxb);
-                if (R > 0 && z1 >= 0 && z1 < GD) visit(z1, cxa, cxb);
-            }
-            if (R > 0) {
-                const int za = max(z0 + 1, 0), zb = min(z1 - 1, GD - 1);
-                for (int cz = za; cz <= zb; cz++) {
-                    if (x0 >= 0 && x0 < GD) visit(cz, x0, x0);
-                    if (x1 >= 0 && x1 < GD) visit(cz, x1, x1);
-                }
-            }
-            if (x0 <= 0 && z0 <= 0 && x1 >= GD - 1 && z1 >= GD - 1) break;
-            float lb = INFINITY;
-            if (x0 > 0) lb = fminf(lb, ux - (H.x0 + (float)x0 * H.cs));
-            if (x1 < GD - 1) lb = fminf(lb, (H.x0 + (float)(x1 + 1) * H.cs) - ux);
-            if (z0 > 0) lb = fminf(lb, uz - (H.z0 + (float)z0 * H.cs));
-            if (z1 < GD - 1) lb = fminf(lb, (H.z0 + (float)(z1 + 1) * H.cs) - uz);
-            lb = lb * 0.999f - 1e-4f * H.cs;
-            if (lb > 0.0f && b3 < lb * lb) break;
-        }
-    }
-    const size_t o = ((size_t)b * n + i) * 3;
-    *reinterpret_cast<Trip<float>*>(dist2 + o) = Trip<float>{b1, b2, b3};
-    *reinterpret_cast<Trip<int32_t>*>(idx + o) = Trip<int32_t>{i1, i2, i3};
-    if (weight) {
-        float r0 = 1.0f / (sqrtf(b1) + 1e-8f);
-        float r1 = 1.0f / (sqrtf(b2) + 1e-8f);
-        float r2 = 1.0f / (sqrtf(b3) + 1e-8f);
-        float s = (r0 + r1) + r2;
-        *reinterpret_cast<Trip<float>*>(weight + o) = Trip<float>{r0 / s, r1 / s, r2 / s};
+    if (!finite_q) return;
+    const float fx = (ux - H.x0) * H.inv_cs, fz = (uz - H.z0) * H.inv_cs;
+    const int qcx = (int)floorf(fminf(fmaxf(fx, -1.0f), (float)GD)), qcz = (int)floorf(fminf(fmaxf(fz, -1.0f), (float)GD));
+    for (int R = 0;; R++) {
+        const int x0 = qcx - R, x1 = qcx + R, z0 = qcz - R, z1 = qcz + R;
+        const int cxa = max(x0, 0), cxb = min(x1, GD - 1);
+        visit2(cxa <= cxb && z0 >= 0 && z0 < GD, z0, cxa, cxb,
+               cxa <= cxb && R > 0 && z1 >= 0 && z1 < GD, z1, cxa, cxb);
+        if (R > 0) {
+            const int za = max(z0 + 1, 0), zb = min(z1 - 1, GD - 1);
+            const bool okl = x0 >= 0 && x0 < GD, okr = x1 >= 0 && x1 < GD;
+            if (okl || okr)
+                for (int cz = za; cz <= zb; cz++) visit2(okl, cz, x0, x0, okr, cz, x1, x1);
+        }
+        if (x0 <= 0 && z0 <= 0 && x1 >= GD - 1 && z1 >= GD - 1) break;
+        float lb = INFINITY;
+        if (x0 > 0) lb = fminf(lb, ux - (H.x0 + (float)x0 * H.cs));
+        if (x1 < GD - 1) lb = fminf(lb, (H.x0 + (float)(x1 + 1) * H.cs) - ux);
+        if (z0 > 0) lb = fminf(lb, uz - (H.z0 + (float)z0 * H.cs));
+        if (z1 < GD - 1) lb = fminf(lb, (H.z0 + (float)(z1 + 1) * H.cs) - uz);
+        lb = lb * 0.999f - 1e-4f * H.cs;
+        if (lb > 0.0f && b3 < lb * lb) break;
+    }
+}
+
+__global__ __launch_bounds__(GNN_LDS_THREADS) void grid_three_nn_kernel(const void* __restrict__ grid, size_t fb,
+                                                                        const float* __restrict__ unknown, int n, int qpb, int lds_m,
+                                                                        float* __restrict__ dist2, int32_t* __restrict__ idx,
+                                                                        float* __restrict__ weight) {
+    extern __shared__ __attribute__((aligned(16))) char gsm[];
+    const int b = blockIdx.y, tid = threadIdx.x;
+    const GridHeader H = *grid_header(grid, fb, b);
+    const int32_t* __restrict__ cstart = grid_cells(grid, fb, b);
+    const float4* __restrict__ pts = grid_points(grid, fb, b);
+    float4* spts = reinterpret_cast<float4*>(gsm);
+    int32_t* scell = reinterpret_cast<int32_t*>(gsm + (size_t)lds_m * sizeof(float4));
+    const bool staged = lds_m != 0 && H.dim == GNN_LDS_DIM;
+    if (staged) {
+        for (int t = tid; t < lds_m; t += blockDim.x) spts[t] = pts[t];
+        const int4* csrc = reinterpret_cast<const int4*>(cstart);
+        int4* cdst = reinterpret_cast<int4*>(scell);
+        for (int t = tid; t < GNN_LDS_DIM * GNN_LDS_DIM / 4; t += blockDim.x) cdst[t] = csrc[t];
+        if (tid == 0) scell[GNN_LDS_DIM * GNN_LDS_DIM] = cstart[GNN_LDS_DIM * GNN_LDS_DIM];
+        __syncthreads();
+    }
+    const int qend = min(n, (blockIdx.x + 1) * qpb);
+    for (int i = blockIdx.x * qpb + tid; i < qend; i += blockDim.x) {
+        const float* u = unknown + ((size_t)b * n + i) * 3;
+        const float ux = u[0], uy = u[1], uz = u[2];
+        float b1 = INFINITY, b2 = INFINITY, b3 = INFINITY;
+        int i1 = 0, i2 = 0, i3 = 0;
+        if (staged) grid_three_nn_rings(H, scell, spts, ux, uy, uz, b1, b2, b3, i1, i2, i3);
+        else grid_three_nn_rings(H, cstart, pts, ux, uy, uz, b1, b2, b3, i1, i2, i3);
+        const size_t o = ((size_t)b * n + i) * 3;
+        *reinterpret_cast<Trip<float>*>(dist2 + o) = Trip<float>{b1, b2, b3};
+        *reinterpret_cast<Trip<int32_t>*>(idx + o) = Trip<int32_t>{i1, i2, i3};
+        if (weight) {
+            float r0 = 1.0f / (sqrtf(b1) + 1e-8f);
+            float r1 = 1.0f / (sqrtf(b2) + 1e-8f);
+            float r2 = 1.0f / (sqrtf(b3) + 1e-8f);
+            float s = (r0 + r1) + r2;
+            *reinterpret_cast<Trip<float>*>(weight + o) = Trip<float>{r0 / s, r1 / s, r2 / s};
+        }
     }
 }
 
@@ -276,19 +327,18 @@
     PRCNN_REQUIRE(B >= 0 && N > 0 && M >= 0 && nsample_a > 0 && nsample_b >= 0, "prcnn_ball_query2_grid: bad shape");
     if (B == 0 || M == 0) return PRCNN_OK;
     PRCNN_REQUIRE(grid && new_xyz && idx_a && (!dual || idx_b), "prcnn_ball_query2_grid: null pointer");
-    const size_t lds = (size_t)(nsample_a + nsample_b) * GBQ_THREADS * sizeof(int);
+    size_t lds = (size_t)(nsample_a + nsample_b) * GBQ_THREADS * sizeof(int);
     PRCNN_REQUIRE(lds <= 64 * 1024, "prcnn_ball_query2_grid: nsample %d+%d too large for the LDS hit lists", nsample_a, nsample_b);
+    if (xyz && lds < NB_CHUNK_BYTES) lds = NB_CHUNK_BYTES;
     dim3 g(prcnn_divup(M, GBQ_THREADS), B);
     const float r2a = radius_a * radius_a, r2b = radius_b * radius_b;
     if (dual)
         hipLaunchKernelGGL(grid_ball_query_kernel<true>, g, dim3(GBQ_THREADS), lds, (hipStream_t)stream, grid, grid_frame_bytes(N),
-                           new_xyz, M, radius_a, r2a, nsample_a, idx_a, radius_b, r2b, nsample_b, idx_b, N, xyz ? 1 : 0);
+                           xyz, new_xyz, M, radius_a, r2a, nsample_a, idx_a, radius_b, r2b, nsample_b, idx_b, N);
     else
         hipLaunchKernelGGL(grid_ball_query_kernel<false>, g, dim3(GBQ_THREADS), lds, (hipStream_t)stream, grid, grid_frame_bytes(N),
-                           new_xyz, M, radius_a, r2a, nsample_a, idx_a, 0.f, 0.f, 0, (int32_t*)nullptr, N, xyz ? 1 : 0);
+                           xyz, new_xyz, M, radius_a, r2a, nsample_a, idx_a, 0.f, 0.f, 0, (int32_t*)nullptr, N);
     PRCNN_LAUNCH_CHECK("prcnn_ball_query2_grid");
-    if (xyz) return prcnn_launch_ball_query_scan(xyz, new_xyz, B, N, M, radius_a, nsample_a, idx_a, radius_b, nsample_b, idx_b, grid,
-                                                 (hipStream_t)stream);
     return PRCNN_OK;
 }
 
@@ -297,8 +347,19 @@
     PRCNN_REQUIRE(B >= 0 && n >= 0 && m > 0, "prcnn_three_nn_grid: bad shape B=%d n=%d m=%d", B, n, m);
     if (B == 0 || n == 0) return PRCNN_OK;
     PRCNN_REQUIRE(grid && unknown && dist2 && idx, "prcnn_three_nn_grid: null pointer");
-    hipLaunchKernelGGL(grid_three_nn_kernel, dim3(prcnn_divup(n, GNN_THREADS), B), dim3(GNN_THREADS), 0, (hipStream_t)stream, grid,
-                       grid_frame_bytes(m), unknown, n, dist2, idx, weight);
+    int threads = GNN_THREADS, qpb = GNN_THREADS, lds_m = 0;
+    if (m <= GNN_LDS_MAX_M && ((uintptr_t)grid & 15) == 0) {
+        static PrcnnLdsLimit attr;
+        if (!attr.raise((const void*)grid_three_nn_kernel, GNN_LDS_MAX_M * 16 + GNN_LDS_CELL_BYTES))
+            return prcnn_fail(PRCNN_EHIP, "prcnn_three_nn_grid: cannot raise the dynamic LDS limit");
+        threads = GNN_LDS_THREADS;
+        while (threads > GNN_THREADS && (long)B * prcnn_divup(n, threads) < 256) threads >>= 1;
+        qpb = threads;
+        if (threads == GNN_LDS_THREADS && (long)B * prcnn_divup(n, 2 * threads) >= 256) qpb = 2 * threads;
+        lds_m = m;
+    }
+    hipLaunchKernelGGL(grid_three_nn_kernel, dim3(prcnn_divup(n, qpb), B), dim3(threads), lds_m ? (size_t)lds_m * 16 + GNN_LDS_CELL_BYTES : 0,
+                       (hipStream_t)stream, grid, grid_frame_bytes(m), unknown, n, qpb, lds_m, dist2, idx, weight);
     PRCNN_LAUNCH_CHECK("prcnn_three_nn_grid");
     return PRCNN_OK;
 }
diff --git a/pointrcnn_amd/csrc/grid_layout.h b/pointrcnn_amd/csrc/grid_layout.h
--- a/pointrcnn_amd/csrc/grid_layout.h
+++ b/pointrcnn_amd/csrc/grid_layout.h
@@ -18,5 +18,104 @@
 __device__ __forceinline__ const GridHeader* grid_header(const void* g, size_t fb, int b) { return (const GridHeader*)((const char*)g + fb * b); }
 __device__ __forceinline__ bool grid_frame_dense(const GridHeader& H, int N) { return H.cand > (float)N * (1.0f / 32.0f); }
 
-int prcnn_launch_ball_query_scan(const float* xyz, const float* new_xyz, int B, int N, int M, float radius_a, int nsample_a,
-                                 int32_t* idx_a, float radius_b, int nsample_b, int32_t* idx_b, const void* grid, hipStream_t s);
+#define BQ_THREADS 64
+#define NB_CHUNK 1024
+#define NB_CHUNK_BYTES (NB_CHUNK * 16)
+
+typedef float f32x2 __attribute__((ext_vector_type(2)));
+
+__device__ __forceinline__ f32x2 pair_sqdist(const float* rec, f32x2 qx, f32x2 qy, f32x2 qz) {
+    float4 a = *reinterpret_cast<const float4*>(rec);
+    f32x2 z = *reinterpret_cast<const f32x2*>(rec + 4);
+    f32x2 dx = qx - (f32x2){a.x, a.y}, dy = qy - (f32x2){a.z, a.w}, dz = qz - z;
+    return (dx * dx + dy * dy) + dz * dz;
+}
+
+__device__ __forceinline__ int chunk_scan_len(int count, int c0, int step = 8) { return (min(NB_CHUNK, count - c0) + step - 1) & ~(step - 1); }
+
+template <typename T> struct __attribute__((packed, aligned(4))) Trip { T a, b, c; };
+
+template <bool DUAL>
+__device__ __forceinline__ void ball_query_scan_block(float* spts, const float* __restrict__ xyz, const float* __restrict__ new_xyz,
+                                                      int N, int M, int b, int mblock, float r2a, int nsa, int32_t* __restrict__ idxa,
+                                                      float r2b, int nsb, int32_t* __restrict__ idxb) {
+    const int tid = threadIdx.x;
+    const int m = mblock * BQ_THREADS + tid;
+    const bool valid = m < M;
+    const float* __restrict__ p = xyz + (size_t)b * N * 3;
+    float qx = 0.f, qy = 0.f, qz = 0.f;
+    if (valid) {
+        const float* q = new_xyz + ((size_t)b * M + m) * 3;
+        qx = q[0]; qy = q[1]; qz = q[2];
+    }
+    const f32x2 qx2 = {qx, qx}, qy2 = {qy, qy}, qz2 = {qz, qz};
+    int32_t* oa = idxa + ((size_t)b * M + (valid ? m : 0)) * nsa;
+    int32_t* ob = DUAL ? idxb + ((size_t)b * M + (valid ? m : 0)) * nsb : nullptr;
+    int cnta = 0, cntb = 0, firsta = 0, firstb = 0;
+    const float r2max = DUAL ? fmaxf(r2a, r2b) : r2a;
+    bool done = !valid;
+
+    constexpr int PER_LANE = NB_CHUNK * 3 / BQ_THREADS;
+    float pre[PER_LANE];
+    auto fetch_chunk = [&](int c0) {
+        const int cnt3 = min(NB_CHUNK, N - c0) * 3, len3 = chunk_scan_len(N, c0) * 3;
+        const float* src = p + (size_t)c0 * 3;
+#pragma unroll
+        for (int u = 0; u < PER_LANE; u++) {
+            int i = tid + u * BQ_THREADS;
+            if (u * BQ_THREADS < len3) pre[u] = i < cnt3 ? src[i] : INFINITY;
+        }
+    };
+    auto store_chunk = [&](int c0) {
+        const int len3 = chunk_scan_len(N, c0) * 3;
+#pragma unroll
+        for (int u = 0; u < PER_LANE; u++) {
+            int i = tid + u * BQ_THREADS;
+            int pt = i / 3, c = i - pt * 3;
+            if (i < len3) spts[(pt >> 1) * 8 + c * 2 + (pt & 1)] = pre[u];
+        }
+    };
+    fetch_chunk(0);
+    for (int c0 = 0; c0 < N; c0 += NB_CHUNK) {
+        if (__all(done)) break;
+        __syncthreads();
+        store_chunk(c0);
+        __syncthreads();
+        if (c0 + NB_CHUNK < N) fetch_chunk(c0 + NB_CHUNK);
+        if (!done) {
+            const int len = chunk_scan_len(N, c0);
+            for (int i0 = 0; i0 < len; i0 += 8) {
+                f32x2 d2[4];
+                bool any = false;
+#pragma unroll
+                for (int u = 0; u < 4; u++) {
+                    d2[u] = pair_sqdist(spts + (i0 / 2 + u) * 8, qx2, qy2, qz2);
+                    any |= (d2[u].x < r2max) | (d2[u].y < r2max);
+                }
+                if (any) {
+#pragma unroll
+                    for (int u = 0; u < 8; u++) {
+                        float d = (u & 1) ? d2[u >> 1].y : d2[u >> 1].x;
+                        if (d < r2max) {
+                            int k = c0 + i0 + u;
+                            if (d < r2a && cnta < nsa) {
+                                if (cnta == 0) firsta = k;
+                                oa[cnta++] = k;
+                            }
+                            if (DUAL && d < r2b && cntb < nsb) {
+                                if (cntb == 0) firstb = k;
+                                ob[cntb++] = k;
+                            }
+                        }
+                    }
+                    if (cnta >= nsa && (!DUAL || cntb >= nsb)) { done = true; break; }
+                }
+            }
+        }
+    }
+    if (valid) {
+        for (int s = cnta; s < nsa; s++) oa[s] = firsta;
+        if (DUAL)
+            for (int s = cntb; s < nsb; s++) ob[s] = firstb;
+    }
+}
diff --git a/pointrcnn_amd/csrc/neighbor.hip b/pointrcnn_amd/csrc/neighbor.hip
--- a/pointrcnn_amd/csrc/neighbor.hip
+++ b/pointrcnn_amd/csrc/neighbor.hip
@@ -1,29 +1,26 @@
 #include "grid_layout.h"
 
-#define BQ_THREADS 64
 #define NN_THREADS 256
-#define NB_CHUNK 1024
-
-typedef float f32x2 __attribute__((ext_vector_type(2)));
-
-__device__ __forceinline__ f32x2 pair_sqdist(const float* rec, f32x2 qx, f32x2 qy, f32x2 qz) {
-    float4 a = *reinterpret_cast<const float4*>(rec);
-    f32x2 z = *reinterpret_cast<const f32x2*>(rec + 4);
-    f32x2 dx = qx - (f32x2){a.x, a.y}, dy = qy - (f32x2){a.z, a.w}, dz = qz - z;
-    return (dx * dx + dy * dy) + dz * dz;
-}
 
 template <bool DUAL>
 __global__ __launch_bounds__(BQ_THREADS) void ball_query_kernel(const float* __restrict__ xyz,
                                                                 const float* __restrict__ new_xyz, int N, int M,
                                                                 float r2a, int nsa, int32_t* __restrict__ idxa,
-                                                                float r2b, int nsb, int32_t* __restrict__ idxb,
-                                                                const void* __restrict__ grid, size_t grid_fb) {
+                                                                float r2b, int nsb, int32_t* __restrict__ idxb) {
     __shared__ __attribute__((aligned(16))) float spts[NB_CHUNK * 4];
-    const int b = blockIdx.y, tid = threadIdx.x;
-    if (grid && !grid_frame_dense(*grid_header(grid, grid_fb, b), N)) return;
-    const int m = blockIdx.x * BQ_THREADS + tid;
+    ball_query_scan_block<DUAL>(spts, xyz, new_xyz, N, M, blockIdx.y, blockIdx.x, r2a, nsa, idxa, r2b, nsb, idxb);
+}
+
+template <bool DUAL, int L>
+__global__ __launch_bounds__(BQ_THREADS) void ball_query_lanes_kernel(const float* __restrict__ xyz,
+                                                                      const float* __restrict__ new_xyz, int N, int M, int seg_log2,
+                                                                      float r2a, int nsa, int32_t* __restrict__ idxa,
+                                                                      float r2b, int nsb, int32_t* __restrict__ idxb) {
+    __shared__ __attribute__((aligned(16))) float spts[(NB_CHUNK / 2 + L) * 8];
+    const int b = blockIdx.y, tid = threadIdx.x, l = tid & (L - 1);
+    const int m = blockIdx.x * (BQ_THREADS / L) + tid / L;
     const bool valid = m < M;
+    const int seg = 1 << seg_log2, chunk = seg * L;
     const float* __restrict__ p = xyz + (size_t)b * N * 3;
     float qx = 0.f, qy = 0.f, qz = 0.f;
     if (valid) {
@@ -33,80 +30,104 @@
     const f32x2 qx2 = {qx, qx}, qy2 = {qy, qy}, qz2 = {qz, qz};
     int32_t* oa = idxa + ((size_t)b * M + (valid ? m : 0)) * nsa;
     int32_t* ob = DUAL ? idxb + ((size_t)b * M + (valid ? m : 0)) * nsb : nullptr;
-    int cnta = 0, cntb = 0, firsta = 0, firstb = 0;
+    int basea = 0, baseb = 0, firsta = 0, firstb = 0;
     const float r2max = DUAL ? fmaxf(r2a, r2b) : r2a;
     bool done = !valid;
 
     constexpr int PER_LANE = NB_CHUNK * 3 / BQ_THREADS;
     float pre[PER_LANE];
     auto fetch_chunk = [&](int c0) {
-        const int cnt3 = min(NB_CHUNK, N - c0) * 3;
+        const int cnt = min(chunk, N - c0), cnt3 = cnt * 3, len3 = ((cnt + 7) & ~7) * 3;
         const float* src = p + (size_t)c0 * 3;
 #pragma unroll
         for (int u = 0; u < PER_LANE; u++) {
             int i = tid + u * BQ_THREADS;
-            pre[u] = i < cnt3 ? src[i] : INFINITY;
+            if (u * BQ_THREADS < len3) pre[u] = i < cnt3 ? src[i] : INFINITY;
         }
     };
-    auto store_chunk = [&]() {
+    fetch_chunk(0);
+    for (int c0 = 0; c0 < N; c0 += chunk) {
+        if (__all(done)) break;
+        const int len = (min(chunk, N - c0) + 7) & ~7;
+        __syncthreads();
 #pragma unroll
         for (int u = 0; u < PER_LANE; u++) {
             int i = tid + u * BQ_THREADS;
-            int pt = i / 3, c = i - pt * 3;
-            spts[(pt >> 1) * 8 + c * 2 + (pt & 1)] = pre[u];
-        }
-    };
-    fetch_chunk(0);
-    for (int c0 = 0; c0 < N; c0 += NB_CHUNK) {
-        if (__all(done)) break;
+            int pt = i / 3, c = i - pt * 3, pr = pt >> 1;
+            if (i < len * 3) spts[(pr + (pr >> (seg_log2 - 1))) * 8 + c * 2 + (pt & 1)] = pre[u];
+        }
         __syncthreads();
-        store_chunk();
-        __syncthreads();
-        if (c0 + NB_CHUNK < N) fetch_chunk(c0 + NB_CHUNK);
+        if (c0 + chunk < N) fetch_chunk(c0 + chunk);
+        unsigned long long ma = 0, mb = 0;
         if (!done) {
-            for (int i0 = 0; i0 < NB_CHUNK; i0 += 8) {
+            const float* rec = spts + l * ((seg >> 1) + 1) * 8;
+            for (int i0 = 0; i0 < seg && l * seg + i0 < len; i0 += 8) {
                 f32x2 d2[4];
                 bool any = false;
 #pragma unroll
                 for (int u = 0; u < 4; u++) {
-                    d2[u] = pair_sqdist(spts + (i0 / 2 + u) * 8, qx2, qy2, qz2);
+                    d2[u] = pair_sqdist(rec + (i0 / 2 + u) * 8, qx2, qy2, qz2);
                     any |= (d2[u].x < r2max) | (d2[u].y < r2max);
                 }
                 if (any) {
+                    unsigned ha = 0, hb = 0;
 #pragma unroll
                     for (int u = 0; u < 8; u++) {
                         float d = (u & 1) ? d2[u >> 1].y : d2[u >> 1].x;
-                        if (d < r2max) {
-                            int k = c0 + i0 + u;
-                            if (d < r2a && cnta < nsa) {
-                                if (cnta == 0) firsta = k;
-                                oa[cnta++] = k;
-                            }
-                            if (DUAL && d < r2b && cntb < nsb) {
-                                if (cntb == 0) firstb = k;
-                                ob[cntb++] = k;
-                            }
-                        }
+                        ha |= (unsigned)(d < r2a) << u;
+                        if (DUAL) hb |= (unsigned)(d < r2b) << u;
                     }
-                    if (cnta >= nsa && (!DUAL || cntb >= nsb)) { done = true; break; }
+                    ma |= (unsigned long long)ha << i0;
+                    mb |= (unsigned long long)hb << i0;
                 }
             }
         }
+        const int ca = __popcll(ma), cb = __popcll(mb);
+        int inca = ca, incb = cb;
+#pragma unroll
+        for (int d = 1; d < L; d <<= 1) {
+            const int ua = __shfl_up(inca, d, L), ub = DUAL ? __shfl_up(incb, d, L) : 0;
+            if (l >= d) { inca += ua; incb += ub; }
+        }
+        int offa = basea + inca - ca, offb = baseb + incb - cb;
+        basea += __shfl(inca, L - 1, L);
+        if (DUAL) baseb += __shfl(incb, L - 1, L);
+        const int k0 = c0 + l * seg;
+        while (ma && offa < nsa) {
+            const int k = k0 + __ffsll(ma) - 1;
+            ma &= ma - 1;
+            if (offa == 0) firsta = k;
+            oa[offa++] = k;
+        }
+        while (DUAL && mb && offb < nsb) {
+            const int k = k0 + __ffsll(mb) - 1;
+            mb &= mb - 1;
+            if (offb == 0) firstb = k;
+            ob[offb++] = k;
+        }
+        done = !valid || (basea >= nsa && (!DUAL || baseb >= nsb));
+    }
+#pragma unroll
+    for (int s = 1; s < L; s <<= 1) {
+        firsta |= __shfl_xor(firsta, s, 64);
+        if (DUAL) firstb |= __shfl_xor(firstb, s, 64);
     }
     if (valid) {
-        for (int s = cnta; s < nsa; s++) oa[s] = firsta;
+        for (int s = min(basea, nsa) + l; s < nsa; s += L) oa[s] = firsta;
         if (DUAL)
-            for (int s = cntb; s < nsb; s++) ob[s] = firstb;
-    }
-}
-
+            for (int s = min(baseb, nsb) + l; s < nsb; s += L) ob[s] = firstb;
+    }
+}
+
+
+template <int L>
 __global__ __launch_bounds__(NN_THREADS) void three_nn_kernel(const float* __restrict__ unknown,
                                                               const float* __restrict__ known, int n, int m,
                                                               float* __restrict__ dist2, int32_t* __restrict__ idx,
                                                               float* __restrict__ weight) {
     __shared__ __attribute__((aligned(16))) float spts[NB_CHUNK * 4];
-    const int b = blockIdx.y, tid = threadIdx.x;
-    const int i = blockIdx.x * NN_THREADS + tid;
+    const int b = blockIdx.y, tid = threadIdx.x, l = tid & (L - 1);
+    const int i = blockIdx.x * (NN_THREADS / L) + tid / L;
     const bool valid = i < n;
     const float* __restrict__ p = known + (size_t)b * m * 3;
     float ux = 0.f, uy = 0.f, uz = 0.f;
@@ -120,31 +141,32 @@
     constexpr int PER_LANE = NB_CHUNK * 3 / NN_THREADS;
     float pre[PER_LANE];
     auto fetch_chunk = [&](int c0) {
-        const int cnt3 = min(NB_CHUNK, m - c0) * 3;
+        const int cnt3 = min(NB_CHUNK, m - c0) * 3, len3 = chunk_scan_len(m, c0, 8 * L) * 3;
         const float* src = p + (size_t)c0 * 3;
 #pragma unroll
         for (int u = 0; u < PER_LANE; u++) {
             int e = tid + u * NN_THREADS;
-            pre[u] = e < cnt3 ? src[e] : INFINITY;
+            if (u * NN_THREADS < len3) pre[u] = e < cnt3 ? src[e] : INFINITY;
         }
     };
     fetch_chunk(0);
     for (int c0 = 0; c0 < m; c0 += NB_CHUNK) {
+        const int len = chunk_scan_len(m, c0, 8 * L);
         __syncthreads();
 #pragma unroll
         for (int u = 0; u < PER_LANE; u++) {
             int e = tid + u * NN_THREADS;
             int pt = e / 3, c = e - pt * 3;
-            spts[(pt >> 1) * 8 + c * 2 + (pt & 1)] = pre[u];
+            if (e < len * 3) spts[(pt >> 1) * 8 + c * 2 + (pt & 1)] = pre[u];
         }
         __syncthreads();
         if (c0 + NB_CHUNK < m) fetch_chunk(c0 + NB_CHUNK);
-        for (int j0 = 0; j0 < NB_CHUNK; j0 += 8) {
+        for (int p0 = l; p0 < (len >> 1); p0 += 4 * L) {
             f32x2 d[4];
             bool any = false;
 #pragma unroll
             for (int u = 0; u < 4; u++) {
-                d[u] = pair_sqdist(spts + (j0 / 2 + u) * 8, ux2, uy2, uz2);
+                d[u] = pair_sqdist(spts + (p0 + u * L) * 8, ux2, uy2, uz2);
                 any |= (d[u].x < b3) | (d[u].y < b3);
             }
             if (any) {
@@ -152,7 +174,7 @@
                 for (int u = 0; u < 8; u++) {
                     float dd = (u & 1) ? d[u >> 1].y : d[u >> 1].x;
                     if (dd < b3) {
-                        int k = c0 + j0 + u;
+                        int k = c0 + 2 * (p0 + (u >> 1) * L) + (u & 1);
                         if (dd < b1) { b3 = b2; i3 = i2; b2 = b1; i2 = i1; b1 = dd; i1 = k; }
                         else if (dd < b2) { b3 = b2; i3 = i2; b2 = dd; i2 = k; }
                         else { b3 = dd; i3 = k; }
@@ -161,42 +183,89 @@
             }
         }
     }
-    if (valid) {
-        size_t o = ((size_t)b * n + i) * 3;
-        dist2[o] = b1; dist2[o + 1] = b2; dist2[o + 2] = b3;
-        idx[o] = i1; idx[o + 1] = i2; idx[o + 2] = i3;
+    if (L > 1) {
+        float r[3];
+        int ri[3];
+#pragma unroll
+        for (int t = 0; t < 3; t++) {
+            float d = b1;
+            int k = i1;
+#pragma unroll
+            for (int s = 1; s < L; s <<= 1) {
+                const float od = __shfl_xor(d, s, 64);
+                const int ok = __shfl_xor(k, s, 64);
+                const bool lt = od < d || (od == d && ok < k);
+                d = lt ? od : d; k = lt ? ok : k;
+            }
+            r[t] = d; ri[t] = k;
+            if (d < INFINITY && b1 == d && i1 == k) { b1 = b2; i1 = i2; b2 = b3; i2 = i3; b3 = INFINITY; i3 = 0; }
+        }
+        b1 = r[0]; b2 = r[1]; b3 = r[2];
+        i1 = ri[0]; i2 = ri[1]; i3 = ri[2];
+    }
+    if (valid && l == 0) {
+        const size_t o = ((size_t)b * n + i) * 3;
+        *reinterpret_cast<Trip<float>*>(dist2 + o) = Trip<float>{b1, b2, b3};
+        *reinterpret_cast<Trip<int32_t>*>(idx + o) = Trip<int32_t>{i1, i2, i3};
         if (weight) {
             float r0 = 1.0f / (sqrtf(b1) + 1e-8f);
             float r1 = 1.0f / (sqrtf(b2) + 1e-8f);
             float r2 = 1.0f / (sqrtf(b3) + 1e-8f);
             float s = (r0 + r1) + r2;
-            weight[o] = r0 / s; weight[o + 1] = r1 / s; weight[o + 2] = r2 / s;
-        }
-    }
+            *reinterpret_cast<Trip<float>*>(weight + o) = Trip<float>{r0 / s, r1 / s, r2 / s};
+        }
+    }
+}
+
+static int lanes_per_query(long queries, int candidates) {
+    if (queries >= 65536) return 1;
+    int L = 8;
+    while (L < 64 && queries * L < 131072) L <<= 1;
+    while (L > 8 && L * 8 > candidates) L >>= 1;
+    return L;
+}
+
+template <int L>
+static void launch_ball_query_lanes(const float* xyz, const float* new_xyz, int B, int N, int M, int seg_log2, float r2a, int nsa,
+                                    int32_t* ia, float r2b, int nsb, int32_t* ib, bool dual, hipStream_t s) {
+    dim3 grid(prcnn_divup(M, BQ_THREADS / L), B);
+    if (dual)
+        hipLaunchKernelGGL((ball_query_lanes_kernel<true, L>), grid, dim3(BQ_THREADS), 0, s, xyz, new_xyz, N, M, seg_log2, r2a, nsa, ia,
+                           r2b, nsb, ib);
+    else
+        hipLaunchKernelGGL((ball_query_lanes_kernel<false, L>), grid, dim3(BQ_THREADS), 0, s, xyz, new_xyz, N, M, seg_log2, r2a, nsa, ia,
+                           0.f, 0, (int32_t*)nullptr);
 }
 
 static int ball_query_impl(const float* xyz, const float* new_xyz, int B, int N, int M, float ra, int nsa, int32_t* ia,
-                           float rb, int nsb, int32_t* ib, bool dual, hipStream_t s, const void* dense_grid = nullptr) {
+                           float rb, int nsb, int32_t* ib, bool dual, hipStream_t s) {
     PRCNN_REQUIRE(B >= 0 && N > 0 && M >= 0 && nsa > 0 && (!dual || nsb > 0),
                   "prcnn_ball_query: bad shape B=%d N=%d M=%d nsample=%d/%d", B, N, M, nsa, nsb);
     if (B == 0 || M == 0) return PRCNN_OK;
     PRCNN_REQUIRE(xyz && new_xyz && ia && (!dual || ib), "prcnn_ball_query: null pointer");
+    float r2a = ra * ra, r2b = rb * rb;
+    const int L = lanes_per_query((long)B * M, N);
+    if (L > 1) {
+        int seg_log2 = 3;
+        while (seg_log2 < 6 && (L << seg_log2) < N && (L << seg_log2) < NB_CHUNK) seg_log2++;
+        switch (L) {
+            case 8: launch_ball_query_lanes<8>(xyz, new_xyz, B, N, M, seg_log2, r2a, nsa, ia, r2b, nsb, ib, dual, s); break;
+            case 16: launch_ball_query_lanes<16>(xyz, new_xyz, B, N, M, seg_log2, r2a, nsa, ia, r2b, nsb, ib, dual, s); break;
+            case 32: launch_ball_query_lanes<32>(xyz, new_xyz, B, N, M, seg_log2, r2a, nsa, ia, r2b, nsb, ib, dual, s); break;
+            default: launch_ball_query_lanes<64>(xyz, new_xyz, B, N, M, seg_log2, r2a, nsa, ia, r2b, nsb, ib, dual, s); break;
+        }
+        PRCNN_LAUNCH_CHECK("prcnn_ball_query");
+        return PRCNN_OK;
+    }
     dim3 grid(prcnn_divup(M, BQ_THREADS), B);
-    float r2a = ra * ra, r2b = rb * rb;
-    const size_t gfb = grid_frame_bytes(N);
     if (dual)
         hipLaunchKernelGGL(ball_query_kernel<true>, grid, dim3(BQ_THREADS), 0, s, xyz, new_xyz, N, M, r2a, nsa, ia, r2b,
-                           nsb, ib, dense_grid, gfb);
+                           nsb, ib);
     else
         hipLaunchKernelGGL(ball_query_kernel<false>, grid, dim3(BQ_THREADS), 0, s, xyz, new_xyz, N, M, r2a, nsa, ia,
-                           0.f, 0, (int32_t*)nullptr, dense_grid, gfb);
+                           0.f, 0, (int32_t*)nullptr);
     PRCNN_LAUNCH_CHECK("prcnn_ball_query");
     return PRCNN_OK;
-}
-
-int prcnn_launch_ball_query_scan(const float* xyz, const float* new_xyz, int B, int N, int M, float radius_a, int nsample_a,
-                                 int32_t* idx_a, float radius_b, int nsample_b, int32_t* idx_b, const void* grid, hipStream_t s) {
-    return ball_query_impl(xyz, new_xyz, B, N, M, radius_a, nsample_a, idx_a, radius_b, nsample_b, idx_b, nsample_b > 0, s, grid);
 }
 
 PRCNN_API int prcnn_ball_query(const float* xyz, const float* new_xyz, int B, int N, int M, float radius, int nsample,
@@ -211,13 +280,26 @@
                            (hipStream_t)stream);
 }
 
+template <int L>
+static void launch_three_nn(const float* unknown, const float* known, int B, int n, int m, float* dist2, int32_t* idx,
+                            float* weight, hipStream_t s) {
+    hipLaunchKernelGGL(three_nn_kernel<L>, dim3(prcnn_divup(n, NN_THREADS / L), B), dim3(NN_THREADS), 0, s, unknown, known, n, m,
+                       dist2, idx, weight);
+}
+
 PRCNN_API int prcnn_three_nn(const float* unknown, const float* known, int B, int n, int m, float* dist2, int32_t* idx,
                              float* weight, prcnn_stream_t stream) {
     PRCNN_REQUIRE(B >= 0 && n >= 0 && m > 0, "prcnn_three_nn: bad shape B=%d n=%d m=%d", B, n, m);
     if (B == 0 || n == 0) return PRCNN_OK;
     PRCNN_REQUIRE(unknown && known && dist2 && idx, "prcnn_three_nn: null pointer");
-    hipLaunchKernelGGL(three_nn_kernel, dim3(prcnn_divup(n, NN_THREADS), B), dim3(NN_THREADS), 0, (hipStream_t)stream,
-                       unknown, known, n, m, dist2, idx, weight);
+    hipStream_t s = (hipStream_t)stream;
+    switch (lanes_per_query((long)B * n, m)) {
+        case 1: launch_three_nn<1>(unknown, known, B, n, m, dist2, idx, weight, s); break;
+        case 8: launch_three_nn<8>(unknown, known, B, n, m, dist2, idx, weight, s); break;
+        case 16: launch_three_nn<16>(unknown, known, B, n, m, dist2, idx, weight, s); break;
+        case 32: launch_three_nn<32>(unknown, known, B, n, m, dist2, idx, weight, s); break;
+        default: launch_three_nn<64>(unknown, known, B, n, m, dist2, idx, weight, s); break;
+    }
     PRCNN_LAUNCH_CHECK("prcnn_three_nn");
     return PRCNN_OK;
 }
diff --git a/pointrcnn_amd/opbench.py b/pointrcnn_amd/opbench.py
--- a/pointrcnn_amd/opbench.py
+++ b/pointrcnn_amd/opbench.py
@@ -455,6 +455,18 @@
     emit("ball_query2", "B%d N%d M4096 r(.1,.5) ns(16,32)" % (B, N),
          timeit(lambda: ops.ball_query2(0.1, 16, 0.5, 32, xyz, new_xyz)), pairs=B * N * 4096)
     emit("three_nn", "B%d n%d m4096" % (B, N), timeit(lambda: ops.three_nn(xyz, new_xyz)), pairs=B * N * 4096)
+    lv = [new_xyz]
+    for npoint in (1024, 256, 64):
+        lv.append(ops.gather_rows(lv[-1], ops.furthest_point_sample(lv[-1], npoint)))
+    emit("ball_query2 SA3", "B%d N1024 M256 r(1,2) ns(16,32)" % B, timeit(lambda: ops.ball_query2(1.0, 16, 2.0, 32, lv[1], lv[2])), pairs=B * 1024 * 256)
+    emit("ball_query2 SA4", "B%d N256 M64 r(2,4) ns(16,32)" % B, timeit(lambda: ops.ball_query2(2.0, 16, 4.0, 32, lv[2], lv[3])), pairs=B * 256 * 64)
+    emit("three_nn FP2", "B%d n1024 m256" % B, timeit(lambda: ops.three_nn(lv[1], lv[2], want_weight=True)), pairs=B * 1024 * 256)
+    emit("three_nn FP3", "B%d n256 m64" % B, timeit(lambda: ops.three_nn(lv[2], lv[3], want_weight=True)), pairs=B * 256 * 64)
+    R = 16 * B
+    roi_pts = (torch.rand(R, 512, 3, generator=g) * torch.tensor([2.0, 2.0, 4.5])).to(dev)
+    roi_ctr = ops.gather_rows(roi_pts, ops.furthest_point_sample(roi_pts, 128))
+    emit("ball_query RCNN SA1", "B%d N512 M128 r.2 ns64" % R, timeit(lambda: ops.ball_query(0.2, 64, roi_pts, roi_ctr)), pairs=R * 512 * 128)
+    del lv, roi_pts, roi_ctr
 
     feat = torch.randn(B, 96, 4096, device=dev)
     xyz1 = new_xyz
```

Result: faster. 15130 frames/s (median of 6 runs) (+6.7%).
